# luanaruiz9/gated_gcrnns

Hardware: AMD Instinct MI355X
Metric: sequences/sec (node), N=1000 K=5 T=32 F=64 (higher is better)
Workload: dtype bf16

## Files before the change

gated_gcrnns_amd/_lib.py:

```python
import ctypes as C
import os

import torch

from . import build as _build

F32, F64, BF16 = 0, 1, 2

_c_i64 = C.c_int64
_c_p = C.c_void_p


class GcrnnError(RuntimeError):
    pass


def _load():
    path = os.environ.get('GCRNN_LIBPATH')
    if path:
        return _bind(C.CDLL(path))
    path = _build.LIBPATH
    if _build.needs_build() and os.path.exists(_build.HIPCC):
        _build.build(verbose=False)
    if not os.path.exists(path):
        raise ImportError(
            'gated_gcrnns_amd: %s is missing. Build it with `python -m gated_gcrnns_amd.build` '
            '(needs hipcc; there is no CPU fallback).' % path)
    return _bind(C.CDLL(path))


def _bind(lib):
    sig = {
        'gcrnn_version': (C.c_int, []),
        'gcrnn_status_string': (C.c_char_p, [C.c_int]),
        'gcrnn_last_hip_error': (C.c_char_p, []),
        'gcrnn_csr_count': (C.c_int, [_c_p, _c_i64, C.c_int, C.c_int, C.c_double, C.POINTER(_c_i64)]),
        'gcrnn_csr_fill': (C.c_int, [_c_p, _c_i64, C.c_int, C.c_int, C.c_double, _c_p, _c_p, _c_p]),
        'gcrnn_degree_order': (C.c_int, [_c_p, _c_i64, _c_p]),
        'gcrnn_pack_node_major': (C.c_int, [C.c_int, _c_p, _c_p, _c_i64, _c_i64, _c_i64, _c_i64, _c_p, _c_p]),
        'gcrnn_pack_node_major_sum_f32': (C.c_int, [_c_p, _c_p, _c_i64, _c_i64, _c_i64, _c_i64, _c_i64, _c_p]),
        'gcrnn_node_gate_filter_supported': (C.c_int, [_c_i64, _c_i64, _c_i64, C.c_double]),
        'gcrnn_node_gate_filter_f32': (C.c_int, [_c_p, _c_p, _c_i64, _c_i64, _c_i64, _c_i64, _c_i64, _c_i64, _c_p, _c_p, _c_p, _c_i64, C.c_double, _c_p, C.c_int, _c_p]),
        'gcrnn_unpack_node_major': (C.c_int, [C.c_int, _c_p, _c_p, _c_i64, _c_i64, _c_i64, _c_i64, _c_p, _c_p]),
        'gcrnn_spmm': (C.c_int, [C.c_int, _c_i64, _c_p, _c_p, _c_p, _c_p, _c_p, _c_i64, _c_i64, C.c_int, _c_p]),
        'gcrnn_spmm_ex': (C.c_int, [C.c_int, _c_i64, _c_p, _c_p, _c_p, _c_p, _c_p, _c_i64, _c_i64, C.c_int, _c_p, C.c_double, _c_i64,
                                    C.c_int, C.c_int, C.c_int, C.c_int, _c_p]),
        'gcrnn_taps_mfma_supported': (C.c_int, [C.c_int, _c_i64, _c_i64, _c_i64]),
        'gcrnn_taps_mfma_forward': (C.c_int, [C.c_int, _c_p, _c_p, _c_p, _c_p, _c_p, _c_p, _c_i64, _c_i64, _c_i64, _c_i64, _c_i64, _c_i64, _c_p]),
        'gcrnn_taps_bf16_supported': (C.c_int, [_c_i64, _c_i64, _c_i64]),
        'gcrnn_taps_bf16_forward': (C.c_int, [_c_p, _c_p, _c_p, _c_p, _c_p, _c_i64, _c_i64, _c_i64, _c_i64, _c_p]),
        'gcrnn_batch_time_mse_slabs': (_c_i64, [_c_i64, _c_i64]),
        'gcrnn_batch_time_mse': (C.c_int, [C.c_int, _c_p, _c_p, _c_p, _c_p, _c_i64, _c_i64, _c_p]),
        'gcrnn_adam_flat': (C.c_int, [C.c_int, _c_p, _c_p, _c_p, _c_p, _c_i64, C.c_double, C.c_double, C.c_double, C.c_double,
                                      C.c_double, _c_p, _c_p]),
        'gcrnn_adam_flat_dlr': (C.c_int, [C.c_int, _c_p, _c_p, _c_p, _c_p, _c_i64, _c_p, C.c_double, C.c_double, C.c_double,
                                          C.c_double, _c_p, _c_p]),
        'gcrnn_sgd_flat': (C.c_int, [C.c_int, _c_p, _c_p, _c_i64, _c_p, C.c_double, _c_p]),
        'gcrnn_rmsprop_flat': (C.c_int, [C.c_int, _c_p, _c_p, _c_p, _c_i64, _c_p, C.c_double, C.c_double, C.c_double, _c_p]),
        'gcrnn_taps_forward': (C.c_int, [C.c_int, _c_p, _c_p, _c_i64, _c_p, _c_p, C.c_double, _c_p,
                                         _c_i64, _c_i64, _c_i64, _c_i64, C.c_int, _c_p]),
        'gcrnn_taps_backward_data': (C.c_int, [C.c_int, _c_p, _c_p, _c_p, _c_p, _c_i64,
                                               _c_i64, _c_i64, _c_i64, _c_i64, _c_p]),
        'gcrnn_taps_backward_weight_parts': (C.c_int, [_c_i64, _c_i64, _c_i64, _c_i64, C.POINTER(_c_i64), C.POINTER(_c_i64)]),
        'gcrnn_taps_backward_weight': (C.c_int, [C.c_int, _c_p, _c_p, _c_p, _c_i64, _c_p, _c_p, C.c_double,
                                                 _c_i64, _c_i64, _c_i64, _c_i64, _c_p]),
        'gcrnn_ell_size': (C.c_int, [_c_p, _c_i64, _c_p, C.c_int, C.c_int, _c_i64, C.POINTER(_c_i64)]),
        'gcrnn_ell_fill': (C.c_int, [_c_p, _c_p, _c_p, _c_i64, _c_p, C.c_int, C.c_int, _c_i64, _c_p, _c_p, _c_p, _c_p]),
        'gcrnn_ell_assign_rows_z': (C.c_int, [_c_p, _c_p, _c_i64, _c_p, C.c_int, _c_i64, _c_i64, _c_p]),
        'gcrnn_ell_fill_z': (C.c_int, [_c_p, _c_p, _c_p, _c_i64, _c_p, C.c_int, C.c_int, _c_i64, _c_p, _c_i64, _c_p, _c_p, _c_p]),
        'gcrnn_ell_assign_rows': (C.c_int, [_c_p, _c_p, _c_i64, _c_p, C.c_int, _c_i64, _c_p]),
        'gcrnn_fused_supported': (C.c_int, [_c_i64, _c_i64, _c_i64, _c_i64]),
        'gcrnn_fused_padded_nodes': (_c_i64, []),
        'gcrnn_fused_step_waves': (_c_i64, []),
        'gcrnn_fused_wgrad_waves': (_c_i64, []),
        'gcrnn_pack_seq_major': (C.c_int, [C.c_int, _c_p, _c_p, _c_i64, _c_i64, _c_i64, _c_i64, _c_i64, _c_p, _c_p]),
        'gcrnn_pack_seq_major_padded': (C.c_int, [_c_p, _c_p] + [_c_i64] * 6 + [_c_p]),
        'gcrnn_unpack_seq_major': (C.c_int, [C.c_int, _c_p, _c_p, _c_i64, _c_i64, _c_i64, _c_i64, _c_i64, _c_p, _c_p]),
        'gcrnn_fused_pack_weights': (C.c_int, [C.c_int, _c_p, _c_p, _c_p, _c_i64, _c_i64, _c_i64, _c_i64, _c_p]),
        'gcrnn_fused_forward_bf16': (C.c_int, [_c_p, _c_p, _c_p, _c_p, _c_p, _c_p, _c_p, _c_p, _c_p, _c_p, _c_p,
                                               _c_p, _c_p,
                                               _c_i64, _c_i64, _c_i64, _c_i64, _c_i64, _c_i64, _c_i64, _c_p, C.c_int, _c_p, C.c_double, _c_p, _c_p, _c_p, _c_p]),
        'gcrnn_fused_pack_weights_wide': (C.c_int, [C.c_int, _c_p, _c_p, _c_p, _c_i64, _c_i64, _c_i64, _c_i64, _c_i64, C.c_double, _c_p]),
        'gcrnn_fused_forward_wide_supported': (C.c_int, [_c_i64] * 7 + [C.c_double, C.c_int, C.c_int]),
        'gcrnn_fused_forward_wide_bf16': (C.c_int, [_c_p] * 10 + [_c_i64] * 7 + [_c_p, C.c_int, _c_p, _c_p, _c_p, _c_p]),
        'gcrnn_fused_forward_wide_scratch_bytes': (_c_i64, [_c_i64, _c_i64, C.c_int]),
        'gcrnn_fused_forward_wide_scratch_bf16': (C.c_int, [_c_p] * 3 + [_c_i64] + [_c_p] * 7 + [_c_i64] * 7 + [_c_p, C.c_int, _c_p, _c_p, _c_p, _c_p]),
        'gcrnn_fused_forward_wide_head_supported': (C.c_int, [_c_i64] * 7 + [C.c_double, C.c_int, C.c_int]),
        'gcrnn_fused_forward_wide_head_bf16': (C.c_int, [_c_p] * 3 + [_c_i64] + [_c_p] * 7 + [_c_i64] * 7 + [_c_p] * 7),
        'gcrnn_fused_pack_weights_wide_bias': (C.c_int, [C.c_int] + [_c_p] * 5 + [_c_i64] * 5 + [C.c_double, _c_p]),
        'gcrnn_fused_forward_wide_user_bytes': (_c_i64, [_c_i64] * 3),
        'gcrnn_fused_forward_wide_user_supported': (C.c_int, [_c_i64] * 7 + [C.c_double, C.c_int]),
        'gcrnn_fused_forward_wide_user_bf16': (C.c_int, [_c_p, _c_i64, _c_p, _c_p, _c_i64] + [_c_p] * 5 + [_c_i64] * 7 + [_c_p, C.c_int, _c_p, _c_p, _c_p, _c_p]),
        'gcrnn_fused_forward_wide_head_user_supported': (C.c_int, [_c_i64] * 7 + [C.c_double, C.c_int]),
        'gcrnn_fused_forward_wide_head_user_bf16': (C.c_int, [_c_p, _c_i64, _c_p, _c_p, _c_i64] + [_c_p] * 5 + [_c_i64] * 7 + [_c_p] * 7),
        'gcrnn_fused_backward_data_wide_supported': (C.c_int, [_c_i64] * 6 + [C.c_double, C.c_int, C.c_int]),
        'gcrnn_fused_backward_data_wide_bf16': (C.c_int, [_c_p] * 8 + [_c_i64] * 6 + [_c_p] * 7),
        'gcrnn_fused_backward_data_wide_head_supported': (C.c_int, [_c_i64] * 6 + [C.c_double, C.c_int]),
        'gcrnn_fused_backward_data_wide_head_bf16': (C.c_int, [_c_p] * 9 + [_c_i64] * 6 + [_c_p] * 4),
        'gcrnn_gate_readout_finish': (C.c_int, [_c_p, _c_i64, _c_p, _c_p, _c_p, _c_p, _c_i64, _c_p]),
        'gcrnn_fused_filter_output_wide_supported': (C.c_int, [_c_i64] * 7 + [C.c_double, C.c_int, C.c_int]),
        'gcrnn_fused_filter_output_wide_bf16': (C.c_int, [_c_p] * 7 + [_c_i64] * 7 + [_c_p, _c_p]),
        'gcrnn_fused_node_forward_wide_supported': (C.c_int, [_c_i64] * 6 + [C.c_double, C.c_int]),
        'gcrnn_fused_node_forward_wide_bf16': (C.c_int, [_c_p] * 11 + [_c_i64] * 6 + [_c_p, C.c_int, _c_p]),
        'gcrnn_fused_gate_pair_wide_supported': (C.c_int, [_c_i64] * 7 + [C.c_double, C.c_int, C.c_int]),
        'gcrnn_fused_gate_pair_prepass_wide_bf16': (C.c_int, [_c_p] * 12 + [_c_i64] * 7 + [_c_p, _c_p, _c_p, _c_p]),
        'gcrnn_fused_gate_pair_prepass_taps_wide_bf16': (C.c_int, [_c_p] * 7 + [_c_i64] + [_c_p] * 5 + [_c_i64] * 7 + [_c_p, _c_p, _c_p, _c_p]),
        'gcrnn_fused_inline_pack_supported': (C.c_int, [_c_i64, _c_i64, _c_i64, _c_i64, _c_i64, C.c_double]),
        'gcrnn_fused_seq_steps_per_launch': (_c_i64, [_c_i64] * 7 + [C.c_double, C.c_int, C.c_int, C.c_int]),
        'gcrnn_fused_filter_output_bf16': (C.c_int, [_c_p] * 11 + [_c_i64] * 7 + [C.c_double, C.c_int, _c_p]),
        'gcrnn_fused_node_forward_bf16': (C.c_int, [_c_p] * 15 + [_c_i64] * 6 + [_c_p, C.c_int, C.c_double, _c_p]),
        'gcrnn_fused_node_backward_data_bf16': (C.c_int, [_c_p] * 12 + [_c_i64] * 6 + [C.c_double, _c_p, C.c_int, _c_p]),
        'gcrnn_node_cell_backward': (C.c_int, [_c_p] * 11 + [_c_i64] * 5 + [_c_p]),
        'gcrnn_node_gate_dot': (C.c_int, [_c_p, _c_p, _c_p, _c_i64, _c_i64, _c_i64, _c_i64, _c_i64, _c_p]),
        'gcrnn_node_gate_dot_backward': (C.c_int, [_c_p, _c_p, _c_p, _c_p, _c_i64, _c_i64, _c_i64, _c_i64, _c_i64, _c_p]),
        'gcrnn_fused_edge_attention_supported': (C.c_int, [_c_i64, _c_i64]),
        'gcrnn_fused_edge_attention_bf16': (C.c_int, [_c_p] * 13 + [_c_i64] * 5 + [C.c_double, _c_p]),
        'gcrnn_fused_edge_attention_backward_supported': (C.c_int, [_c_i64, _c_i64, _c_i64]),
        'gcrnn_fused_edge_attention_backward_bf16': (C.c_int, [_c_p] * 14 + [_c_i64] * 6 + [C.c_double, _c_p]),
        'gcrnn_fused_backward_step_bf16': (C.c_int, [_c_p] * 11 + [_c_i64] * 5 + [C.c_double, _c_p, _c_p, _c_i64, C.c_int, _c_p]),
        'gcrnn_fused_backward_seed_bf16': (C.c_int, [_c_p, _c_p, _c_p, _c_i64, _c_p]),
        'gcrnn_fused_x3_supported': (C.c_int, [_c_i64, _c_i64, _c_i64, _c_i64, _c_i64]),
        'gcrnn_pack_seq_major_x3': (C.c_int, [_c_p, _c_p, _c_i64, _c_i64, _c_i64, _c_i64, _c_i64, _c_p]),
        'gcrnn_fused_pack_weights_x3': (C.c_int, [_c_p, _c_p, _c_p, _c_i64, _c_i64, _c_i64, _c_i64, _c_p]),
        'gcrnn_fused_forward_x3': (C.c_int, [_c_p] * 8 + [_c_i64] * 7 + [C.c_double, _c_p, C.c_int, _c_p, _c_p]),
        'gcrnn_fused_forward_x3_scaled': (C.c_int, [_c_p] * 9 + [_c_i64] * 7 + [C.c_double, _c_p, _c_i64, _c_p, _c_p]),
        'gcrnn_fused_x3_training_supported': (C.c_int, [_c_i64] * 5),
        'gcrnn_fused_backward_data_x3': (C.c_int, [_c_p] * 8 + [_c_i64] * 6 + [C.c_double, _c_p, _c_p]),
        'gcrnn_fused_backward_weight_f32': (C.c_int, [_c_p] * 9 + [_c_i64] * 7 + [C.c_double, _c_p, _c_p]),
        'gcrnn_fused_backward_data_x3_gated': (C.c_int, [_c_p] * 8 + [_c_i64] * 6 + [C.c_double, _c_p, _c_p, _c_p, _c_p, _c_p]),
        'gcrnn_fused_filter_x3': (C.c_int, [_c_p] * 6 + [_c_i64] * 5 + [C.c_double, _c_p, _c_p]),
        'gcrnn_fused_backward_weight_f32_gated': (C.c_int, [_c_p] * 9 + [_c_i64] * 7 + [C.c_double, _c_p, _c_p, C.c_int, _c_p, _c_p]),
        'gcrnn_fused_gate_cells_x3': (C.c_int, [_c_p] * 8 + [_c_i64] * 7 + [C.c_double, _c_p, C.c_int, _c_p, _c_p]),
        'gcrnn_pack_seq_major_x3_ex': (C.c_int, [_c_p, _c_p] + [_c_i64] * 5 + [_c_p, _c_p, C.c_int, _c_i64, _c_p]),
        'gcrnn_x3_item_dots': (C.c_int, [_c_p] * 5 + [_c_i64] * 4 + [_c_p]),
        'gcrnn_x3_node_gate_step': (C.c_int, [_c_p] * 7 + [_c_i64] * 5 + [_c_p]),
        'gcrnn_pack_seq_major_steps': (C.c_int, [_c_p, _c_p, _c_i64, _c_i64, _c_i64, _c_i64, _c_i64, _c_i64, _c_i64, _c_i64, _c_p]),
        'gcrnn_fused_gate_prepass_bf16': (C.c_int, [_c_p, _c_p, _c_p, _c_p, _c_p, _c_p, _c_p, _c_p, _c_p, _c_p, _c_p, _c_p, _c_p,
                                                    _c_i64, _c_i64, _c_i64, _c_i64, _c_i64, _c_i64, _c_i64, _c_p, C.c_double, C.c_int, _c_p]),
        'gcrnn_fused_gate_prepass_pack_bf16': (C.c_int, [_c_p] * 14 + [_c_i64] * 7 + [_c_p, C.c_double, C.c_int, _c_p]),
        'gcrnn_fused_gate_prepass_lays_out': (_c_i64, [_c_i64] * 7 + [C.c_double, C.c_int]),
        'gcrnn_fused_gate_prepass_taps_bf16': (C.c_int, [_c_p] * 7 + [_c_i64] + [_c_p] * 7 + [_c_i64] * 7 + [_c_p, C.c_double, C.c_int, _c_p]),
        'gcrnn_fused_gate_prepass_taps_supported': (C.c_int, [_c_i64] * 7 + [C.c_double, C.c_int, C.c_int, _c_i64]),
        'gcrnn_fused_gate_readout_slabs': (_c_i64, [_c_i64]),
        'gcrnn_all_zero_flag_bf16': (C.c_int, [_c_p, _c_i64, _c_p, _c_p]),
        'gcrnn_fused_gate_readout_backward_bf16': (C.c_int, [_c_p, _c_p, _c_p, _c_p, _c_i64, _c_i64, _c_i64, _c_p]),
        'gcrnn_fused_gate_grad_bf16': (C.c_int, [_c_p] * 12 + [_c_i64] * 7 + [C.c_double, C.c_int, _c_p]),
        'gcrnn_fused_backward_data_bf16': (C.c_int, [_c_p, _c_p, _c_p, _c_p, _c_p, _c_p, _c_p, _c_p, _c_p, _c_p, _c_p,
                                                     _c_i64, _c_i64, _c_i64, _c_i64, _c_i64, _c_i64, _c_p, _c_p, _c_p, C.c_double, _c_p, C.c_int, _c_p]),
        'gcrnn_fused_wgrad_slots': (_c_i64, [_c_i64, _c_i64]),
        'gcrnn_fused_wgrad_bf16_slots': (_c_i64, [_c_i64, _c_i64, _c_i64, _c_i64, C.c_int]),
        'gcrnn_fused_backward_weight_bf16': (C.c_int, [_c_p, _c_p, _c_p, _c_p, _c_p, _c_p, _c_p, _c_p, _c_p, _c_p,
                                                       _c_i64, _c_i64, _c_i64, _c_i64, _c_i64, _c_i64, _c_i64, _c_p, _c_p,
                                                       C.c_int, _c_p, C.c_double, _c_p, _c_p, _c_p]),
        'gcrnn_small_supported': (C.c_int, [C.c_int, _c_i64, _c_i64, _c_i64, _c_i64, _c_i64, _c_i64]),
        'gcrnn_small_forward': (C.c_int, [C.c_int, _c_p, _c_p, _c_p, _c_p, _c_p, _c_p, _c_p, _c_p, _c_p, _c_p, _c_p,
                                          _c_i64, _c_i64, _c_i64, _c_i64, _c_i64, _c_i64, _c_i64, _c_i64, _c_p]),
        'gcrnn_small_backward_supported': (C.c_int, [C.c_int, _c_i64, _c_i64, _c_i64, _c_i64, _c_i64, _c_i64]),
        'gcrnn_small_backward': (C.c_int, [C.c_int] + [_c_p] * 21 + [_c_i64] * 8 + [_c_p]),
        'gcrnn_small_backward_dx': (C.c_int, [C.c_int] + [_c_p] * 22 + [_c_i64] * 8 + [_c_p]),
        'gcrnn_small_dense_supported': (C.c_int, [C.c_int, _c_i64, _c_i64, _c_i64, _c_i64, _c_i64, C.c_int, C.c_int]),
        'gcrnn_small_dense_forward': (C.c_int, [C.c_int] + [_c_p] * 9 + [_c_i64] * 10 + [_c_p]),
        'gcrnn_small_dense_backward': (C.c_int, [C.c_int] + [_c_p] * 16 + [_c_i64] * 10 + [_c_p]),
        'gcrnn_small_dense_backward_dx_supported': (C.c_int, [C.c_int, _c_i64, _c_i64, _c_i64, _c_i64, _c_i64, C.c_int]),
        'gcrnn_small_dense_backward_dx': (C.c_int, [C.c_int] + [_c_p] * 17 + [_c_i64] * 10 + [_c_p]),
        'gcrnn_small_dense_head_supported': (C.c_int, [C.c_int] + [_c_i64] * 6 + [C.c_int] * 3),
        'gcrnn_small_dense_forward_head': (C.c_int, [C.c_int] + [_c_p] * 12 + [_c_i64] * 11 + [C.c_int, _c_p]),
        'gcrnn_small_dense_backward_head': (C.c_int, [C.c_int] + [_c_p] * 18 + [_c_i64] * 11 + [_c_p]),
        'gcrnn_small_dense_node_head_supported': (C.c_int, [C.c_int] + [_c_i64] * 6 + [C.c_int] * 3),
        'gcrnn_small_dense_forward_node_head': (C.c_int, [C.c_int] + [_c_p] * 12 + [_c_i64] * 11 + [C.c_int, _c_p]),
        'gcrnn_small_dense_backward_node_head': (C.c_int, [C.c_int] + [_c_p] * 18 + [_c_i64] * 11 + [_c_p]),
        'gcrnn_small_dense_gnn_head_supported': (C.c_int, [C.c_int] + [_c_i64] * 6 + [C.c_int] * 3),
        'gcrnn_small_dense_forward_gnn_head': (C.c_int, [C.c_int] + [_c_p] * 12 + [_c_i64] * 11 + [C.c_int, C.c_int, _c_p]),
        'gcrnn_small_gnn_head_adjoint': (C.c_int, [C.c_int] + [_c_p] * 4 + [_c_i64] * 3 + [C.c_int, _c_p]),
        'gcrnn_small_gates_supported': (C.c_int, [C.c_int, _c_i64, _c_i64, _c_i64, _c_i64, _c_i64, C.c_int]),
        'gcrnn_small_gates_forward': (C.c_int, [C.c_int] + [_c_p] * 9 + [_c_i64] * 7 + [_c_p]),
        'gcrnn_small_gates_backward': (C.c_int, [C.c_int] + [_c_p] * 14 + [_c_i64] * 7 + [_c_p]),
        'gcrnn_small_gates_backward_dx': (C.c_int, [C.c_int] + [_c_p] * 15 + [_c_i64] * 7 + [_c_p]),
        'gcrnn_small_node_gates_supported': (C.c_int, [C.c_int, _c_i64, _c_i64, _c_i64, _c_i64, _c_i64, C.c_int]),
        'gcrnn_small_node_gates_forward': (C.c_int, [C.c_int] + [_c_p] * 9 + [_c_i64] * 7 + [_c_p]),
        'gcrnn_small_node_gates_backward': (C.c_int, [C.c_int] + [_c_p] * 14 + [_c_i64] * 7 + [_c_p]),
        'gcrnn_small_node_gates_backward_dx': (C.c_int, [C.c_int] + [_c_p] * 15 + [_c_i64] * 7 + [_c_p]),
        'gcrnn_small_edge_supported': (C.c_int, [C.c_int] + [_c_i64] * 7),
        'gcrnn_small_edge_forward': (C.c_int, [C.c_int] + [_c_p] * 21 + [_c_i64] * 9 + [C.c_int, _c_p]),
        'gcrnn_small_edge_backward_supported': (C.c_int, [C.c_int] + [_c_i64] * 7),
        'gcrnn_small_edge_backward': (C.c_int, [C.c_int] + [_c_p] * 33 + [_c_i64] * 9 + [_c_p]),
        'gcrnn_small_edge_backward_dx': (C.c_int, [C.c_int] + [_c_p] * 34 + [_c_i64] * 9 + [_c_p]),
        'gcrnn_small_edge_head_supported': (C.c_int, [C.c_int] + [_c_i64] * 7 + [C.c_int, _c_i64, C.c_int]),
        'gcrnn_small_edge_forward_head': (C.c_int, [C.c_int] + [_c_p] * 24 + [_c_i64] * 10 + [C.c_int, C.c_int, _c_p]),
        'gcrnn_small_edge_backward_head': (C.c_int, [C.c_int] + [_c_p] * 35 + [_c_i64] * 10 + [C.c_int, _c_p]),
        'gcrnn_node_linear_blocks': (_c_i64, [_c_i64, _c_i64]),
        'gcrnn_node_linear_forward': (C.c_int, [C.c_int, _c_p, _c_p, _c_p, _c_p, _c_i64, _c_i64, _c_i64, _c_i64, _c_p]),
        'gcrnn_node_linear_backward': (C.c_int, [C.c_int, _c_p, _c_p, _c_p, _c_p, _c_p, _c_p, _c_i64, _c_i64, _c_i64, _c_i64, _c_p]),
        'gcrnn_node_linear_bf16_supported': (C.c_int, [_c_i64, _c_i64, _c_i64]),
        'gcrnn_node_linear_bf16_blocks': (_c_i64, [_c_i64, _c_i64]),
        'gcrnn_node_linear_bf16_forward': (C.c_int, [C.c_int, _c_p, _c_p, _c_p, _c_p, _c_i64, _c_i64, _c_i64, _c_i64, _c_p]),
        'gcrnn_node_linear_bf16_backward': (C.c_int, [C.c_int, _c_p, _c_p, _c_p, _c_p, _c_p, _c_p, _c_i64, _c_i64, _c_i64, _c_i64, _c_p]),
        'gcrnn_graph_filter_layer_supported': (C.c_int, [C.c_int] + [_c_i64] * 6 + [C.c_int]),
        'gcrnn_graph_filter_layer_wgrad_slots': (_c_i64, [C.c_int] + [_c_i64] * 6 + [C.c_int]),
        'gcrnn_graph_filter_layer_forward': (C.c_int, [C.c_int] + [_c_p] * 7 + [C.c_double] + [_c_i64] * 7 + [C.c_int, _c_p]),
        'gcrnn_graph_filter_layer_backward': (C.c_int, [C.c_int] + [_c_p] * 7 + [_c_i64] + [_c_p] * 3 + [C.c_double] + [_c_i64] * 7
                                              + [C.c_int, _c_p]),
        'gcrnn_rnn_supported': (C.c_int, [C.c_int] + [_c_i64] * 4),
        'gcrnn_rnn_wgrad_slots': (_c_i64, [C.c_int] + [_c_i64] * 4),
        'gcrnn_rnn_forward': (C.c_int, [C.c_int] + [_c_p] * 7 + [_c_i64] * 4 + [C.c_int, _c_p]),
        'gcrnn_rnn_backward': (C.c_int, [C.c_int] + [_c_p] * 10 + [_c_i64] * 5 + [C.c_int, _c_p]),
        'gcrnn_l1_loss_blocks': (_c_i64, [_c_i64]),
        'gcrnn_l1_loss': (C.c_int, [C.c_int, _c_p, _c_p, _c_p, _c_p, _c_i64, C.c_double, _c_p]),
        'gcrnn_scale_unless_one': (C.c_int, [C.c_int, _c_p, _c_p, _c_i64, _c_p]),
        'gcrnn_cross_entropy_blocks': (_c_i64, [_c_i64, _c_i64]),
        'gcrnn_cross_entropy': (C.c_int, [C.c_int] + [_c_p] * 7 + [_c_i64, _c_i64, C.c_double, _c_p]),
        'gcrnn_attention_forward': (C.c_int, [C.c_int] + [_c_p] * 11 + [_c_i64] * 5 + [C.c_double, _c_p]),
        'gcrnn_attention_backward': (C.c_int, [C.c_int] + [_c_p] * 15 + [_c_i64] * 5 + [C.c_double, _c_p]),
        'gcrnn_ell_conflict_cycles': (C.c_int, [_c_p, _c_i64, _c_p, C.POINTER(_c_i64)]),
        'gcrnn_ell_pack_lds': (C.c_int, [_c_p, _c_p, _c_i64, _c_p, _c_p, _c_p]),
    }
    for name, (res, args) in sig.items():
        fn = getattr(lib, name)
        fn.restype = res
        fn.argtypes = args
    return lib, sorted(sig)


lib, EXPORTS = _load()


def check(status, what=''):
    if status != 0:
        detail = lib.gcrnn_last_hip_error().decode() if status == 5 else ''
        raise GcrnnError('%s failed: %s (status %d) %s' % (what or 'gcrnn call', lib.gcrnn_status_string(status).decode(),
                                                        status, detail))


def dtype_code(torch_dtype):
    import torch
    try:
        return {torch.float32: F32, torch.float64: F64, torch.bfloat16: BF16}[torch_dtype]
    except KeyError:
        raise GcrnnError('unsupported dtype %s (float32, float64, bfloat16)' % torch_dtype)
```

gated_gcrnns_amd/csrc/gcrnn_fused_seq32.h:

```cpp
#pragma once

#if defined(GCRNN_SEQ_STAMPS)
static __device__ unsigned long long gcrnn_seq32_stamps[256 * 96];
static __device__ __forceinline__ void gcrnn_stamp32_put(uint32_t lds_addr) {
  const unsigned long long tv = __builtin_amdgcn_s_memtime();
  asm volatile("ds_write_b64 %0, %1" ::"v"(lds_addr), "v"(tv) : "memory");
}
static __device__ __forceinline__ unsigned long long gcrnn_stamp32_get(uint32_t lds_addr) {
  unsigned long long tv;
  asm volatile("ds_read_b64 %0, %1\n\ts_waitcnt lgkmcnt(0)" : "=v"(tv) : "v"(lds_addr) : "memory");
  return tv;
}
#define GCRNN_STAMP32(slot)                                                                                   \
  do {                                                                                                        \
    if (wave == 0 && stamp_on && lane_now() == 0) gcrnn_stamp32_put((uint32_t)reinterpret_cast<uintptr_t>(smem) + M::FLAG_OFF + 8 * (slot)); \
  } while (0)
#define GCRNN_STAMP32_WAVE(slot0)                                                                             \
  do {                                                                                                        \
    if (stamp_on && lane_now() == 0) gcrnn_stamp32_put((uint32_t)reinterpret_cast<uintptr_t>(smem) + M::FLAG_OFF + 8 * ((slot0) + wave)); \
  } while (0)
#define GCRNN_STAMP32_FLUSH()                                                                                 \
  do {                                                                                                        \
    __syncthreads();                                                                                          \
    if (threadIdx.x < 96 && blockIdx.x < 256) gcrnn_seq32_stamps[blockIdx.x * 96 + threadIdx.x] = gcrnn_stamp32_get((uint32_t)reinterpret_cast<uintptr_t>(smem) + M::FLAG_OFF + 8 * threadIdx.x); \
  } while (0)
#ifndef GCRNN_SEQ32_STAMP_READER_NAME
#define GCRNN_SEQ32_STAMP_READER_NAME gcrnn_debug_read_seq32_stamps
#endif
extern "C" int GCRNN_SEQ32_STAMP_READER_NAME(void* host) {
  return hipMemcpyFromSymbol(host, HIP_SYMBOL(gcrnn_seq32_stamps), sizeof(unsigned long long) * 256 * 96) == hipSuccess ? 0 : 1;
}
#else
#define GCRNN_STAMP32_WAVE(slot0) do {} while (0)
#define GCRNN_STAMP32(slot) do {} while (0)
#define GCRNN_STAMP32_FLUSH() do {} while (0)
#endif

#ifndef GCRNN_SEQ32_R1_STREAM_FIRST
#define GCRNN_SEQ32_R1_STREAM_FIRST 0
#endif
#ifndef GCRNN_SEQ32_OPERAND_AT
#define GCRNN_SEQ32_OPERAND_AT 1
#endif
#ifndef GCRNN_SEQ32_NT_ROWS
#define GCRNN_SEQ32_NT_ROWS 0
#endif
#ifndef GCRNN_SEQ32_NT_DMA
#define GCRNN_SEQ32_NT_DMA 0
#endif
#ifndef GCRNN_SEQ32_NT_XLOAD
#define GCRNN_SEQ32_NT_XLOAD 0
#endif
#ifndef GCRNN_SEQ32_NT_STATE
#define GCRNN_SEQ32_NT_STATE 0
#endif
#ifndef GCRNN_SEQ32_NO_ITEM_PREFETCH
#define GCRNN_SEQ32_NO_ITEM_PREFETCH 0
#endif
#ifndef GCRNN_SEQ32_GATED_TAPS_FIRST
#define GCRNN_SEQ32_GATED_TAPS_FIRST 1
#endif
#ifndef GCRNN_SEQ32_YOUNG_PRIO
#define GCRNN_SEQ32_YOUNG_PRIO 0
#endif
#ifndef GCRNN_SEQ32_END_WAIT
#define GCRNN_SEQ32_END_WAIT 0
#endif
#ifndef GCRNN_SEQ32_SAME_ORDER
#define GCRNN_SEQ32_SAME_ORDER 0
#endif

struct Seq32Args {
  const uint16_t* x0; int64_t xstride;
  const uint16_t* hfirst;
  uint16_t* out0; int64_t ostride;
  const uint4* wpack;
  const float* bias;
  const uint16_t* a1; int64_t a1stride;
  int a1_last_only;
  int ubstride;
  const int32_t* tile_nodes; const int32_t* tile_off; const uint2* ell_col4;
  int entries, B, N;
  const uint16_t* pk_src0; int64_t pksrc_stride;
  uint16_t* pk_dst0; int64_t pkdst_stride;
  int pk_stride;
  int nsteps;
  const float* gi0; const float* gf0; int64_t gstride;
  int hmod;
  const int32_t* flags;
  const float* gw;
  const uint4* tapf; float* taps_out; int ntaps;
  float* go;
  uint16_t* out1;
  const uint16_t* dh0_; int64_t dhstride;
  const uint16_t* hs0; int64_t hsstride;
  const float* gsc0; int64_t gscstride;
  float* gpart0; int64_t gpartstride;
  int final_raw;
  uint16_t* final_out; const uint16_t* final_h;
  const float* ng0; int64_t ngstride; int64_t nghalf;
  const float* r1a; const float* r1b;
  int stagger;
  uint16_t* scr;
  const float* head_w; const float* head_b;
  float* y0;
  const uint16_t* h0u; int self_start;
  const uint16_t* dy0; int64_t dystride; int64_t dybstride;
};

__device__ __forceinline__ int lane_now() {
  int ln;
  asm volatile("v_mbcnt_lo_u32_b32 %0, -1, 0\n\tv_mbcnt_hi_u32_b32 %0, -1, %0" : "=v"(ln));
  return ln;
}

#define GCRNN_HOP_ASM_WIDE32_STREAM(D)                                                             \
  do {                                                                                             \
    const int gwbeg = tbeg[0] >> 2, gwend = tend[STILES - 1] >> 2;                                 \
    if (gwbeg < gwend) {                                                                           \
      const int ls_ = lane_now(), r = ls_ & 15, q = ls_ >> 4;                                      \
      const uint32_t colb = lds_col + r * 8 + (q >> 1) * 4;        \
      const uint32_t qh_ = (uint32_t)(q & 1) << 4;                                                 \
      asm volatile(GCRNN_HOP_ASM_WIDE32_TEXT                                                       \
                   : "+v"(D[0][0]), "+v"(D[0][1]), "+v"(D[1][0]), "+v"(D[1][1]), "+v"(D[2][0]), "+v"(D[2][1]), "+v"(D[3][0]), "+v"(D[3][1]), \
                     "+v"(D[4][0]), "+v"(D[4][1]), "+v"(D[5][0]), "+v"(D[5][1]), "+v"(D[6][0]), "+v"(D[6][1]), "+v"(D[7][0]), "+v"(D[7][1])  \
                   : "s"(GCRNN_SGPR(tend[0] >> 2)), "s"(GCRNN_SGPR(tend[1] >> 2)), "s"(GCRNN_SGPR(tend[2] >> 2)), "s"(GCRNN_SGPR(tend[3] >> 2)), \
                     "s"(GCRNN_SGPR(tend[4] >> 2)), "s"(GCRNN_SGPR(tend[5] >> 2)), "s"(GCRNN_SGPR(tend[6] >> 2)), "s"(GCRNN_SGPR(tend[7] >> 2)), \
                     "s"(GCRNN_SGPR(gwbeg)), "s"(GCRNN_SGPR(gwend - 1)), "v"(colb), "v"(qh_)               \
                   : GCRNN_HOP_ASM_WIDE32_CLOBBERS);                                               \
    }                                                                                              \
  } while (0)

template <int K, int HS, int XS>
struct Seq32Map {
  static constexpr int KS = HS + XS;
  static constexpr int PL = GCRNN_HOP_WIDE_PLANE;
  static constexpr int RS2 = 4 * NP + 16;
  static constexpr int BIAS_OFF = PL + 32 * 1024;
  static constexpr int FLAG_OFF = BIAS_OFF + 256;
  static constexpr int WOFF = 2 * PL;
  static constexpr int WB = K * KS * 2048;
  static constexpr int COL_OFF = WOFF + WB;
  static constexpr int NPCK = 128;
  static constexpr int PFS = 256;
  static_assert(16 * RS2 <= BIAS_OFF && FLAG_OFF + 768 <= WOFF, "LDS map");
  static size_t lds_bytes(int64_t entries, bool inline_pack, bool r1 = false) {
    const size_t need = (size_t)COL_OFF + (size_t)entries * 32 + GCRNN_HOP_COLUMN_PAD + NP * 4 + (r1 ? 2 * NP * 4 : 0) + (inline_pack ? (size_t)(32 * (XS > 0 ? XS : HS)) * NPCK * 2 : 0)
                        + PFS;
    return need <= 160 * 1024 ? need : 0;
  }
  static constexpr int HEAD_TAB = 512 + (HS > 1 ? NP * 4 : 0);
  static size_t lds_bytes_head(int64_t entries, bool inline_pack, bool r1 = false) {
    const size_t need = lds_bytes(entries, inline_pack, r1);
    return (need && need + HEAD_TAB <= 160 * 1024) ? need + HEAD_TAB : 0;
  }
};

template <int K, int HS, int XS, int VAR, int MODE = 0, bool GATED = false, bool R1 = false, bool SPLIT = false>
__global__ __launch_bounds__(STHREADS) void fused_seq32_kernel(const Seq32Args a) {
  static_assert(!R1 || !SPLIT, "rank-1 graphs: every mode of the persistent form (the BPTT chain takes the adjoint plan: the factors swap)");
  static_assert(!SPLIT || ((MODE == 0 || MODE == 2) && !R1 && HS > 1), "split sequences: the (un-gated or time-gated) forward and the BPTT chain, with more than one chunk");
  constexpr bool ITEMS = (MODE == 1 || MODE == 3);
  constexpr bool SONLY = (MODE == 2 || MODE == 4);
  constexpr bool PKV = (VAR & 1) != 0, USERV = (VAR & 2) != 0 && (MODE == 0 || MODE == 4);
  constexpr bool SCRV = (VAR & 4) != 0;
  constexpr bool HEADV = (VAR & 8) != 0;
  constexpr bool UPR1 = (VAR & 16) != 0;
  static_assert(!UPR1 || (VAR == 16 && MODE == 2 && !R1 && !SPLIT), "rank-1 upstream: the persistent chain on uniform-weight graphs, no inline pack");
  static_assert(!SCRV || (MODE == 0 && !SPLIT && ((VAR & 2) != 0 || HEADV)), "state scratch: the persistent forward with the user-layout output");
  static_assert(!HEADV || (SCRV && (VAR & 2) == 0), "output head: on the state scratch, no user-layout output");
  constexpr int SCR_CH = NP * 64;
  static_assert(MODE == 0 || ((MODE >= 1 && MODE <= 4) && !GATED), "modes");
  static_assert(MODE < 3 || (!R1 && !SPLIT), "modes 3, 4: uniform-weight graphs, persistent form");
  using M = Seq32Map<K, HS, XS>;
  constexpr int KS = HS + XS;
  constexpr int F = 32 * HS, G = 32 * XS;
  constexpr int NCH = (MODE == 1) ? 2 * HS : HS;
  constexpr int PL = M::PL, WOFF = M::WOFF, WB = M::WB, COL_OFF = M::COL_OFF, RS2 = M::RS2;
  constexpr int NPCK = M::NPCK, NRND = NP / NPCK, NH = NCH * (K - 1), RPH = (NRND + NH - 1) / NH;
  constexpr int PKROWS = SONLY ? F : G;
  static_assert(STILES == 8 && GCRNN_HOP_ASM && K >= 2 && (SONLY ? XS == 0 : XS > 0), "generated hop stream: 8 tiles per wave; the chain's operand is the state alone");
  extern __shared__ __attribute__((aligned(16))) char smem[];
  const int entries = a.entries, B = a.B, N = a.N;

  const int tid = threadIdx.x, lane = tid & 63;
  const int wave = __builtin_amdgcn_readfirstlane(tid >> 6);
  const int r = lane & 15, q = lane >> 4;
  constexpr int NSPL = SPLIT ? HS : 1;
  const int wg_seq = (int)blockIdx.x / NSPL, chunk0 = SPLIT ? (int)blockIdx.x % NSPL : 0, gseq = (int)gridDim.x / NSPL;
  if (wg_seq >= B) return;

  bf16x8 bfr[STILES][KS];
  constexpr bool SELFV = PKV && SCRV && MODE == 0 && !GATED && !SPLIT;
  const bool self_start = SELFV && a.self_start != 0;
  if constexpr (SELFV) {
    if (self_start) {
      constexpr int SROW = NP * 2, SPIECES = 32 * (NP / 8);
      static_assert(32 * SROW <= M::BIAS_OFF && 32 * SROW <= M::WOFF && SPIECES % STHREADS == 0 && NP / 8 == 128, "self-start staging area: below the bias table");
      const int b = wg_seq;
      const int tl = wave * 64 + lane_now();
      int nodes[STILES];
#pragma unroll
      for (int i = 0; i < STILES; ++i) nodes[i] = a.tile_nodes[(wave * STILES + i) * 16 + (tl & 15)] >> 16;
#pragma unroll
      for (int s = 0; s < KS; ++s) {
        const uint16_t* src = s < HS ? a.h0u + (int64_t)b * (F * N) + (int64_t)(32 * s) * N
                                     : a.pk_src0 + (int64_t)b * a.pk_stride + (int64_t)(32 * (s - HS)) * N;
#pragma unroll
        for (int i = 0; i < SPIECES / STHREADS; ++i) {
          const int id = i * STHREADS + tl;
          const int row = id >> 7, cs = id & 127;
          const int col = (cs - 2 * (row >> 3)) & 127;
          if (col * 8 < N)
            __builtin_amdgcn_global_load_lds((const __attribute__((address_space(1))) void*)(src + (int64_t)row * N + col * 8),
                                             (__attribute__((address_space(3))) void*)(smem + (i * STHREADS + wave * 64) * 16), 16, 0, GCRNN_SEQ32_NT_DMA);
        }
        asm volatile("s_waitcnt vmcnt(0)" ::: "memory");
        lds_barrier();
        const int qo = (tl & 63) >> 4;
#pragma unroll
        for (int i = 0; i < STILES; ++i) {
          const bool ok = nodes[i] < N;
          const int nn = ok ? nodes[i] : 0;
          const char* ra = smem + (8 * qo) * SROW + ((((nn >> 3) + 2 * qo) & 127) << 4) + (nn & 7) * 2;
          uint32_t h16[8];
#pragma unroll
          for (int j = 0; j < 8; ++j) h16[j] = *reinterpret_cast<const uint16_t*>(ra + j * SROW);
          typedef __attribute__((__vector_size__(4 * sizeof(unsigned int)))) unsigned int u32x4s_t;
          u32x4s_t v;
#pragma unroll
          for (int jj = 0; jj < 4; ++jj) v[jj] = ok ? (h16[2 * jj] | (h16[2 * jj + 1] << 16)) : 0u;
          bfr[i][s] = __builtin_bit_cast(bf16x8, v);
        }
        lds_barrier();
      }
      if (a.nsteps > 1) {
        constexpr int XN = RPH * NPCK, XROWS = G, XPPR = XN / 8, XPCS = XROWS / 8;
        static_assert(XROWS * XN * 2 <= 32 * SROW && (XROWS * XPPR) % STHREADS == 0 && (XPCS * XN) % STHREADS == 0 && XPPR >= 16, "x_1 start-up rounds");
        const __amdgpu_buffer_rsrc_t rsrc_x1 = __builtin_amdgcn_make_buffer_rsrc(a.pk_dst0 + a.pkdst_stride + (int64_t)b * (NP * G), 0, NP * G * 2, 0x00020000);
        const uint16_t* src = a.pk_src0 + (int64_t)b * a.pk_stride + a.pksrc_stride;
#pragma unroll
        for (int i = 0; i < XROWS * XPPR / STHREADS; ++i) {
          const int id = i * STHREADS + tl;
          const int row = id / XPPR, cs = id - row * XPPR;
          const int col = (cs - 2 * (row >> 3) + XPPR) % XPPR;
          if (col * 8 < N)
            __builtin_amdgcn_global_load_lds((const __attribute__((address_space(1))) void*)(src + (int64_t)row * N + col * 8),
                                             (__attribute__((address_space(3))) void*)(smem + (i * STHREADS + wave * 64) * 16), 16, 0, GCRNN_SEQ32_NT_DMA);
        }
        asm volatile("s_waitcnt vmcnt(0)" ::: "memory");
        lds_barrier();
        constexpr int XRI = XPCS * XN / STHREADS;
        typedef __attribute__((__vector_size__(4 * sizeof(unsigned int)))) unsigned int u32x4x_t;
        u32x4x_t vv[XRI];
#pragma unroll
        for (int i = 0; i < XRI; ++i) {
          const int id = i * STHREADS + tl;
          const int nl = id / XPCS, pc = id - nl * XPCS;
          const char* ra = smem + (8 * pc) * (XN * 2) + ((((nl >> 3) + 2 * pc) % XPPR) << 4) + (nl & 7) * 2;
          uint32_t h16[8];
#pragma unroll
          for (int j = 0; j < 8; ++j) h16[j] = *reinterpret_cast<const uint16_t*>(ra + j * (XN * 2));
          const bool ok = nl < N;
#pragma unroll
          for (int jj = 0; jj < 4; ++jj) vv[i][jj] = ok ? (h16[2 * jj] | (h16[2 * jj + 1] << 16)) : 0u;
        }
#pragma unroll
        for (int i = 0; i < XRI; ++i) asm volatile("" : "+v"(vv[i]));
#pragma unroll
        for (int i = 0; i < XRI; ++i) {
          const int id = i * STHREADS + tl;
          const int nl = id / XPCS, pc = id - nl * XPCS;
          __builtin_amdgcn_raw_buffer_store_b128(vv[i], rsrc_x1, nl * (G * 2) + pc * 16, 0, 0);
        }
        asm volatile("s_waitcnt vmcnt(0)" ::: "memory");
#pragma unroll
        for (int i = 0; i < XRI; ++i) asm volatile("" ::"v"(vv[i]));
        lds_barrier();
      }
    }
  }

  int tbeg[STILES], tend[STILES];
#pragma unroll
  for (int i = 0; i < STILES; ++i) {
    tbeg[i] = a.tile_off[wave * STILES + i];
    tend[i] = a.tile_off[wave * STILES + i + 1];
  }
  char* wtab = smem + COL_OFF + entries * 32 + GCRNN_HOP_COLUMN_PAD;
  for (int idx = tid; idx < NP; idx += STHREADS) reinterpret_cast<int32_t*>(wtab)[idx] = a.tile_nodes[idx];
  [[maybe_unused]] float* r1tab = reinterpret_cast<float*>(wtab + NP * 4);
  if constexpr (R1) {
    for (int idx = tid; idx < NP; idx += STHREADS) {
      const int nd = a.tile_nodes[idx] >> 16;
      r1tab[idx] = nd < NP ? a.r1a[nd] : 0.f;
      r1tab[NP + idx] = nd < NP ? a.r1b[nd] : 0.f;
    }
  }
  auto slot_words = [&](int ln, int (&w)[STILES]) {
    const uint32_t ad = (uint32_t)(COL_OFF + entries * 32 + GCRNN_HOP_COLUMN_PAD) + (uint32_t)((wave * STILES * 16 + (ln & 15)) * 4);
    asm volatile("ds_read_b32 %0, %8\n\tds_read_b32 %1, %8 offset:64\n\tds_read_b32 %2, %8 offset:128\n\tds_read_b32 %3, %8 offset:192\n\t"
                 "ds_read_b32 %4, %8 offset:256\n\tds_read_b32 %5, %8 offset:320\n\tds_read_b32 %6, %8 offset:384\n\tds_read_b32 %7, %8 offset:448\n\t"
                 "s_waitcnt lgkmcnt(0)"
                 : "=&v"(w[0]), "=&v"(w[1]), "=&v"(w[2]), "=&v"(w[3]), "=&v"(w[4]), "=&v"(w[5]), "=&v"(w[6]), "=&v"(w[7])
                 : "v"(ad));
    const int lb = (((ln >> 4) >> 1) << 4) | (((ln >> 4) & 1) << 3);
#pragma unroll
    for (int i = 0; i < STILES; ++i) w[i] ^= lb;
  };
  [[maybe_unused]] auto r1_scale = [&](f32x4 (&ac)[STILES][2], int kind) __attribute__((always_inline)) {
    if constexpr (R1) {
      const uint32_t ad = (uint32_t)(COL_OFF + entries * 32 + GCRNN_HOP_COLUMN_PAD + NP * 4 + NP * 4) + (uint32_t)((wave * STILES * 16 + (lane_now() & 15)) * 4);
      constexpr int NB = (GATED || ITEMS || K == 4) ? 1 : 4;
#pragma unroll
      for (int h4 = 0; h4 < STILES; h4 += NB) {
        float b4[NB];
        if constexpr (NB == 4)
          asm volatile("ds_read_b32 %0, %4\n\tds_read_b32 %1, %4 offset:64\n\tds_read_b32 %2, %4 offset:128\n\tds_read_b32 %3, %4 offset:192\n\t"
                       "s_waitcnt lgkmcnt(0)"
                       : "=&v"(b4[0]), "=&v"(b4[1]), "=&v"(b4[2]), "=&v"(b4[3])
                       : "v"(ad + (uint32_t)(h4 * 64)));
        else
          asm volatile("ds_read_b32 %0, %1\n\ts_waitcnt lgkmcnt(0)" : "=&v"(b4[0]) : "v"(ad + (uint32_t)(h4 * 64)));
#pragma unroll
        for (int e = 0; e < NB; ++e) {
          const float bv = b4[e];
          const float f = kind == 0 ? bv : (bv == 0.f ? 1.f : (kind == 1 ? __builtin_amdgcn_rcpf(bv) : bv));
          ac[h4 + e][0] *= f; ac[h4 + e][1] *= f;
        }
      }
    }
  };

  {
    const int cbytes = entries * 32;
    const char* csrc = reinterpret_cast<const char*>(a.ell_col4);
    for (int p = wave; p * 1024 < cbytes; p += SWAVES)
      if (p * 1024 + lane * 16 < cbytes)
        __builtin_amdgcn_global_load_lds((const __attribute__((address_space(1))) void*)(csrc + p * 1024 + lane * 16),
                                         (__attribute__((address_space(3))) void*)(smem + COL_OFF + p * 1024), 16, 0, 0);
    const char* wsrc = reinterpret_cast<const char*>(a.wpack) + (size_t)chunk0 * WB;
    for (int p = wave; p < WB / 1024; p += SWAVES)
      __builtin_amdgcn_global_load_lds((const __attribute__((address_space(1))) void*)(wsrc + p * 1024 + lane * 16),
                                       (__attribute__((address_space(3))) void*)(smem + WOFF + p * 1024), 16, 0, 0);
    asm volatile("s_waitcnt vmcnt(0)" ::: "memory");
  }
  if (tid < GCRNN_HOP_COLUMN_PAD / 4) reinterpret_cast<uint32_t*>(smem + COL_OFF + entries * 32)[tid] = 0u;
  float* lbias = reinterpret_cast<float*>(smem + M::BIAS_OFF);
  if constexpr (UPR1) {
    if (tid < F) lbias[tid] = a.head_w[tid];
  } else
  if (tid < NCH * 32) lbias[tid] = a.bias ? a.bias[tid] : 0.f;
  if constexpr (HEADV) {
    float* ht = reinterpret_cast<float*>(smem + COL_OFF + entries * 32 + GCRNN_HOP_COLUMN_PAD + NP * 4 + (R1 ? 2 * NP * 4 : 0));
    if (tid < F) ht[tid] = a.head_w[tid];
    if (tid == F) ht[64] = a.head_b ? a.head_b[0] : 0.f;
  }
  __syncthreads();

  if (a.stagger > 0) {
    const unsigned long long t0 = __builtin_amdgcn_s_memtime();
    const unsigned long long d = (unsigned long long)((blockIdx.x >> 3) & 7) * (unsigned long long)a.stagger;
    while (__builtin_amdgcn_s_memtime() - t0 < d) __builtin_amdgcn_s_sleep(16);
  }
  const uint32_t lds0 = (uint32_t)reinterpret_cast<uintptr_t>(smem);
  if (lds0 != 0) __builtin_trap();
  const uint32_t lds_col = lds0 + COL_OFF;
  [[maybe_unused]] float* htab = reinterpret_cast<float*>(wtab + NP * 4 + (R1 ? 2 * NP * 4 : 0));
  char* xtile = wtab + NP * 4 + (R1 ? 2 * NP * 4 : 0) + (HEADV ? M::HEAD_TAB : 0);

  const int skip_hi = __builtin_amdgcn_readfirstlane((MODE == 3 || (MODE == 1 && a.flags && a.flags[0] != 0)) ? 1 : 0);
  const bool skip_h = skip_hi != 0;
  auto load_first_operand = [&](int b) {
    const __amdgpu_buffer_rsrc_t rsrc_h = __builtin_amdgcn_make_buffer_rsrc(const_cast<uint16_t*>(a.hfirst), 0, skip_h ? 0 : (ITEMS ? a.hmod : B) * (NP * F * 2), 0x00020000);
    const __amdgpu_buffer_rsrc_t rsrc_x = __builtin_amdgcn_make_buffer_rsrc(const_cast<uint16_t*>(a.x0), 0, XS > 0 ? B * (NP * G * 2) : 0, 0x00020000);
    const int bh = ITEMS ? __builtin_amdgcn_readfirstlane(b % a.hmod) : b;
    const int ln0 = lane_now(), qo = ln0 >> 4;
    int sw[STILES];
    slot_words(ln0, sw);
#pragma unroll
    for (int s = 0; s < KS; ++s) {
#pragma unroll
      for (int i = 0; i < STILES; ++i) {
        const int w = sw[i];
        if (s < HS)
          bfr[i][s] = __builtin_bit_cast(bf16x8, __builtin_amdgcn_raw_buffer_load_b128(rsrc_h, (w >> 16) * (F * 2) + 16 * qo + 64 * s, bh * (NP * F * 2), 0));
        else
          bfr[i][s] = __builtin_bit_cast(bf16x8, __builtin_amdgcn_raw_buffer_load_b128(rsrc_x, (w >> 16) * (G * 2) + 16 * qo + 64 * (s - HS), b * (NP * G * 2), 0));
      }
    }
  };
  bool have_operand = self_start;
  for (int b = wg_seq; b < B; b += gseq) {
  if (!have_operand) load_first_operand(b);
  have_operand = false;
#pragma unroll 1
  for (int step = 0; step < a.nsteps; ++step) {
    const bool fin = (MODE == 2) && a.final_raw && step == a.nsteps - 1;
    uint16_t* hout = fin ? a.final_out : (a.out0 ? a.out0 + (int64_t)step * a.ostride : nullptr);
    [[maybe_unused]] const uint16_t* ep_dh = (SONLY && !fin && a.dh0_) ? a.dh0_ + (int64_t)step * a.dhstride : nullptr;
    [[maybe_unused]] const float* ep_ng = (MODE == 4) ? a.ng0 + (int64_t)step * a.ngstride : nullptr;
    [[maybe_unused]] const uint16_t* ep_h = (MODE == 2) ? (fin ? a.final_h : (a.hs0 ? a.hs0 + (int64_t)step * a.hsstride : nullptr)) : nullptr;
    [[maybe_unused]] const uint16_t* ep_dy = (UPR1 && !fin && a.dy0) ? a.dy0 + (int64_t)step * a.dystride + (int64_t)b * a.dybstride : nullptr;
    [[maybe_unused]] const bool ep_up = UPR1 ? ep_dy != nullptr : ep_dh != nullptr;
    [[maybe_unused]] float* gpart = (MODE == 2 && a.gpart0) ? a.gpart0 + (int64_t)step * a.gpartstride : nullptr;
    [[maybe_unused]] float gsc = 1.f;
    if constexpr (MODE == 2) {
      if (a.gsc0) gsc = __builtin_bit_cast(float, __builtin_amdgcn_readfirstlane(__builtin_bit_cast(int, a.gsc0[(int64_t)step * a.gscstride + b])));
    }
    float gin = 1.f, gfo = 1.f, gratio = 1.f;
    if constexpr (MODE == 4) {
      if (a.gi0) {
        gin = __builtin_bit_cast(float, __builtin_amdgcn_readfirstlane(__builtin_bit_cast(int, a.gi0[(int64_t)step * a.gstride + b])));
        gfo = __builtin_bit_cast(float, __builtin_amdgcn_readfirstlane(__builtin_bit_cast(int, a.gf0[(int64_t)step * a.gstride + b])));
      }
    }
    if constexpr (GATED) {
      gin = __builtin_bit_cast(float, __builtin_amdgcn_readfirstlane(__builtin_bit_cast(int, a.gi0[(int64_t)step * a.gstride + b])));
      gfo = __builtin_bit_cast(float, __builtin_amdgcn_readfirstlane(__builtin_bit_cast(int, a.gf0[(int64_t)step * a.gstride + b])));
      gratio = __builtin_bit_cast(float, __builtin_amdgcn_readfirstlane(__builtin_bit_cast(int, gfo / fmaxf(gin, 1e-30f))));
    }
    const uint16_t* aux1 = (USERV && a.a1) ? (a.a1_last_only ? (step == a.nsteps - 1 ? a.a1 : nullptr) : a.a1 + (int64_t)step * a.a1stride) : nullptr;
    const bool pk_any = PKV && a.pk_src0 != nullptr;
    const int ubstride = a.ubstride;
    const int nb = b + (int)gridDim.x;
    const int nbq = ITEMS ? __builtin_amdgcn_readfirstlane(nb / a.hmod) : 0, nbr = ITEMS ? __builtin_amdgcn_readfirstlane(nb - nbq * a.hmod) : 0;
    const int64_t pk_soff = ITEMS ? (int64_t)nbr * a.pk_stride + (int64_t)nbq * a.pksrc_stride : (int64_t)b * a.pk_stride;
    const int pk_db = ITEMS ? nb : b;
    const __amdgpu_buffer_rsrc_t rsrc_o = __builtin_amdgcn_make_buffer_rsrc(hout, 0, hout ? B * (NP * F * 2) : 0, 0x00020000);
    [[maybe_unused]] const bool stamp_on = (step == (a.nsteps > 2 ? a.nsteps - 3 : 0)) && b == wg_seq;
    GCRNN_STAMP32(0);
    const bool more = step + 1 < a.nsteps;
    const __amdgpu_buffer_rsrc_t rsrc_xn = __builtin_amdgcn_make_buffer_rsrc(const_cast<uint16_t*>(XS > 0 ? a.x0 + (int64_t)(step + 1) * a.xstride : nullptr), 0, (more && XS > 0) ? B * (NP * G * 2) : 0, 0x00020000);

    f32x4 acc[STILES][2];
    auto taps = [&](int tap, [[maybe_unused]] bool on_sums = false) {
#ifdef GCRNN_SEQ32_EXPERIMENT_NO_HOP_TAPS
      if (tap != K - 1) return;
#endif
      const int ln = lane_now();
      const uint32_t wofs = (uint32_t)WOFF + (uint32_t)ln * 16u;
      if constexpr (GATED) {
        const bool xpart = gin > 1e-30f;
        const bool hpart = !on_sums || gfo > 1e-30f;
        if (on_sums) {
          const float pre = hpart ? 1.f / gfo : (xpart ? 1.f / gin : 1.f);
#pragma unroll
          for (int i = 0; i < STILES; ++i) { acc[i][0] *= pre; acc[i][1] *= pre; }
        }
#pragma unroll
        for (int h = 0; h < 2; ++h) {
          if (hpart) {
#pragma unroll
            for (int s = 0; s < HS; ++s) {
              const bf16x8 afr = __builtin_bit_cast(bf16x8, *reinterpret_cast<const uint4*>(smem + wofs + (uint32_t)(((tap * 2 + h) * KS + s) * 1024)));
#pragma unroll
              for (int i = 0; i < STILES; ++i) acc[i][h] = __builtin_amdgcn_mfma_f32_16x16x32_bf16(afr, bfr[i][s], acc[i][h], 0, 0, 0);
            }
          }
          if (hpart) {
#pragma unroll
            for (int i = 0; i < STILES; ++i) acc[i][h] *= (xpart ? gratio : gfo);
          }
          if (xpart) {
#pragma unroll
            for (int s = HS; s < KS; ++s) {
              const bf16x8 afr = __builtin_bit_cast(bf16x8, *reinterpret_cast<const uint4*>(smem + wofs + (uint32_t)(((tap * 2 + h) * KS + s) * 1024)));
#pragma unroll
              for (int i = 0; i < STILES; ++i) acc[i][h] = __builtin_amdgcn_mfma_f32_16x16x32_bf16(afr, bfr[i][s], acc[i][h], 0, 0, 0);
            }
            if constexpr (GATED) {
#pragma unroll
              for (int i = 0; i < STILES; ++i) acc[i][h] *= gin;
            }
          }
        }
      } else if constexpr (ITEMS) {
#pragma unroll
        for (int h = 0; h < 2; ++h)
#pragma unroll
          for (int s = 0; s < KS; ++s) {
            if (s < HS && skip_h) continue;
            const bf16x8 afr = __builtin_bit_cast(bf16x8, *reinterpret_cast<const uint4*>(smem + wofs + (uint32_t)(((tap * 2 + h) * KS + s) * 1024)));
#pragma unroll
            for (int i = 0; i < STILES; ++i) acc[i][h] = __builtin_amdgcn_mfma_f32_16x16x32_bf16(afr, bfr[i][s], acc[i][h], 0, 0, 0);
          }
      } else {
      uint4 af[2];
      af[0] = *reinterpret_cast<const uint4*>(smem + wofs + (uint32_t)((tap * 2 * KS) * 1024));
#pragma unroll
      for (int hs = 0; hs < 2 * KS; ++hs) {
        const int h = hs / KS, s = hs - h * KS;
        if (hs + 1 < 2 * KS) af[(hs + 1) & 1] = *reinterpret_cast<const uint4*>(smem + wofs + (uint32_t)((tap * 2 * KS + hs + 1) * 1024));
        const bf16x8 afr = __builtin_bit_cast(bf16x8, af[hs & 1]);
#pragma unroll
        for (int i = 0; i < STILES; ++i) acc[i][h] = __builtin_amdgcn_mfma_f32_16x16x32_bf16(afr, bfr[i][s], acc[i][h], 0, 0, 0);
      }
      }
    };
    auto put = [&](auto tpc) __attribute__((always_inline)) {
      constexpr bool tprime = decltype(tpc)::value;
      int sw[STILES];
      slot_words(lane_now(), sw);
#pragma unroll
      for (int i = 0; i < STILES; ++i) {
        const int wv = sw[i];
        if constexpr (R1) {
          const int slot = (wave * STILES + i) * 16 + (lane_now() & 15);
          float av = r1tab[slot];
          if constexpr (tprime) { const float bv = r1tab[NP + slot]; av *= (bv == 0.f ? 1.f : bv); }
          state_put<true>(reinterpret_cast<float*>(smem), wv, acc[i][0] * av);
          state_put<true>(reinterpret_cast<float*>(smem + PL), wv, acc[i][1] * av);
        } else {
          state_put<true>(reinterpret_cast<float*>(smem), wv, acc[i][0]);
          state_put<true>(reinterpret_cast<float*>(smem + PL), wv, acc[i][1]);
        }
      }
    };
    auto seed = [&]() {
#pragma unroll
      for (int i = 0; i < STILES; ++i) { acc[i][0] = f32x4{0.f, 0.f, 0.f, 0.f}; acc[i][1] = f32x4{0.f, 0.f, 0.f, 0.f}; }
      taps(K - 1);
      put(std::false_type{});
    };
    auto seed_taps_beside_rows = [&]() {
#pragma unroll
      for (int i = 0; i < STILES; ++i) { acc[i][0] = f32x4{0.f, 0.f, 0.f, 0.f}; acc[i][1] = f32x4{0.f, 0.f, 0.f, 0.f}; }
      taps(K - 1);
    };
    seed();

#pragma unroll 1
    for (int chunk = chunk0; chunk < (SPLIT ? chunk0 + 1 : NCH); ++chunk) {
      const bool last = SPLIT || chunk == NCH - 1;
      lds_barrier();
      GCRNN_STAMP32(1 + chunk * 24);

      auto pack_target = [&](int v, int& tgt, int& rnd) -> bool {
        if constexpr (ITEMS) {
          rnd = v; tgt = 0;
          return pk_any && v < NRND && nb < B;
        }
        if constexpr (SPLIT) {
          rnd = v; tgt = 0;
          return pk_any && v < NRND;
        }
        if constexpr (MODE == 2) {
          rnd = v; tgt = step + 1;
          return pk_any && v < NRND && tgt < a.nsteps - (a.final_raw ? 1 : 0);
        }
        v += RPH;
        const int wrap = v >= NRND ? 1 : 0;
        rnd = v - wrap * NRND;
        tgt = step + 1 + wrap;
        return pk_any && tgt >= (self_start ? 1 : 2) && tgt < a.nsteps;
      };
      auto pack_issue = [&](int v) {
        int tgt, rnd;
        if (!pack_target(v, tgt, rnd)) return;
        const uint16_t* pk_src = a.pk_src0 + ((ITEMS || SPLIT) ? 0 : (int64_t)tgt * a.pksrc_stride);
        constexpr int PPR = NPCK / 8, PIECES = PKROWS * PPR;
        static_assert(PIECES % STHREADS == 0, "whole pieces per thread");
        const uint16_t* xsrc = pk_src + pk_soff + rnd * NPCK;
        const int tl = wave * 64 + lane_now();
#pragma unroll
        for (int i = 0; i < PIECES / STHREADS; ++i) {
          const int id = i * STHREADS + tl;
          const int row = id / PPR, cs = id - row * PPR;
          const int col = (cs - (row >> 3)) & (PPR - 1);
          if (rnd * NPCK + col * 8 < N)
            __builtin_amdgcn_global_load_lds((const __attribute__((address_space(1))) void*)(xsrc + (int64_t)row * N + col * 8),
                                             (__attribute__((address_space(3))) void*)(xtile + (i * STHREADS + wave * 64) * 16), 16, 0, GCRNN_SEQ32_NT_DMA);
        }
      };
      auto pack_drain = [&](int v) {
        int tgt, rnd;
        if (!pack_target(v, tgt, rnd)) return;
        uint16_t* pk_dst = a.pk_dst0 + ((ITEMS || SPLIT) ? 0 : (int64_t)tgt * a.pkdst_stride);
        constexpr int PCS = PKROWS / 8, RI = PCS * NPCK / STHREADS;
        static_assert(PCS * NPCK % STHREADS == 0, "whole row pieces per thread");
        typedef __attribute__((__vector_size__(4 * sizeof(unsigned int)))) unsigned int u32x4_t;
        const __amdgpu_buffer_rsrc_t rsrc_pk = __builtin_amdgcn_make_buffer_rsrc(pk_dst, 0, B * (NP * PKROWS * 2), 0x00020000);
        const int tl = wave * 64 + lane_now();
        u32x4_t vv[RI];
        static_assert(RI == 1 || RI == 2, "one or two row pieces per thread");
        uint32_t h16[RI][8];
        uint32_t sa[RI];
#pragma unroll
        for (int i = 0; i < RI; ++i) {
          const int id = i * STHREADS + tl;
          const int nl = id / PCS, pc = id - nl * PCS;
          sa[i] = (uint32_t)(xtile - smem) + (uint32_t)((pc * 8) * (NPCK * 2) + ((nl + 8 * pc) & (NPCK - 1)) * 2);
        }
        static_assert(NPCK * 2 == 256, "row pitch of the pack tile in the asm offsets");
        if constexpr (RI == 2) {
          asm volatile("ds_read_u16 %0, %16\n\tds_read_u16 %1, %16 offset:256\n\tds_read_u16 %2, %16 offset:512\n\tds_read_u16 %3, %16 offset:768\n\t"
                       "ds_read_u16 %4, %16 offset:1024\n\tds_read_u16 %5, %16 offset:1280\n\tds_read_u16 %6, %16 offset:1536\n\tds_read_u16 %7, %16 offset:1792\n\t"
                       "ds_read_u16 %8, %17\n\tds_read_u16 %9, %17 offset:256\n\tds_read_u16 %10, %17 offset:512\n\tds_read_u16 %11, %17 offset:768\n\t"
                       "ds_read_u16 %12, %17 offset:1024\n\tds_read_u16 %13, %17 offset:1280\n\tds_read_u16 %14, %17 offset:1536\n\tds_read_u16 %15, %17 offset:1792\n\t"
                       "s_waitcnt lgkmcnt(0)"
                       : "=&v"(h16[0][0]), "=&v"(h16[0][1]), "=&v"(h16[0][2]), "=&v"(h16[0][3]), "=&v"(h16[0][4]), "=&v"(h16[0][5]), "=&v"(h16[0][6]), "=&v"(h16[0][7]),
                         "=&v"(h16[RI - 1][0]), "=&v"(h16[RI - 1][1]), "=&v"(h16[RI - 1][2]), "=&v"(h16[RI - 1][3]), "=&v"(h16[RI - 1][4]), "=&v"(h16[RI - 1][5]), "=&v"(h16[RI - 1][6]), "=&v"(h16[RI - 1][7])
                       : "v"(sa[0]), "v"(sa[RI - 1]));
        } else {
          asm volatile("ds_read_u16 %0, %8\n\tds_read_u16 %1, %8 offset:256\n\tds_read_u16 %2, %8 offset:512\n\tds_read_u16 %3, %8 offset:768\n\t"
                       "ds_read_u16 %4, %8 offset:1024\n\tds_read_u16 %5, %8 offset:1280\n\tds_read_u16 %6, %8 offset:1536\n\tds_read_u16 %7, %8 offset:1792\n\t"
                       "s_waitcnt lgkmcnt(0)"
                       : "=&v"(h16[0][0]), "=&v"(h16[0][1]), "=&v"(h16[0][2]), "=&v"(h16[0][3]), "=&v"(h16[0][4]), "=&v"(h16[0][5]), "=&v"(h16[0][6]), "=&v"(h16[0][7])
                       : "v"(sa[0]));
        }
#pragma unroll
        for (int i = 0; i < RI; ++i) {
          const int id = i * STHREADS + tl;
          const int nl = id / PCS;
          const bool ok = rnd * NPCK + nl < N;
          uint32_t w4[4];
#pragma unroll
          for (int jj = 0; jj < 4; ++jj) w4[jj] = h16[i][2 * jj] | (h16[i][2 * jj + 1] << 16);
          vv[i] = u32x4_t{ok ? w4[0] : 0u, ok ? w4[1] : 0u, ok ? w4[2] : 0u, ok ? w4[3] : 0u};
        }
#pragma unroll
        for (int i = 0; i < RI; ++i) asm volatile("" : "+v"(vv[i]));
#pragma unroll
        for (int i = 0; i < RI; ++i) {
          const int id = i * STHREADS + tl;
          const int nl = id / PCS, pc = id - nl * PCS;
          __builtin_amdgcn_raw_buffer_store_b128(vv[i], rsrc_pk, (rnd * NPCK + nl) * (PKROWS * 2) + pc * 16 + pk_db * (NP * PKROWS * 2), 0, 0);
        }
      };

      auto r0_of = [&](int j) { return (chunk * (K - 1) + (j - 1)) * RPH; };
      auto weights_issue = [&](int wc, int tap) {
        const char* wsrc = reinterpret_cast<const char*>(a.wpack) + (size_t)wc * WB + (size_t)tap * (2 * KS * 1024);
        const int lane = lane_now();
#pragma unroll
        for (int i = 0; i < (2 * KS + SWAVES - 1) / SWAVES; ++i) {
          const int piece = i * SWAVES + wave;
          if (piece < 2 * KS)
            __builtin_amdgcn_global_load_lds((const __attribute__((address_space(1))) void*)(wsrc + piece * 1024 + lane * 16),
                                             (__attribute__((address_space(3))) void*)(smem + WOFF + tap * (2 * KS * 1024) + piece * 1024), 16, 0, 0);
        }
      };
      typedef __attribute__((__vector_size__(4 * sizeof(unsigned int)))) unsigned int u32x4e_t;
      [[maybe_unused]] u32x4e_t eph[MODE == 2 ? STILES : 1], epg[(SONLY && !UPR1) ? STILES : 1];
      [[maybe_unused]] uint32_t epy[UPR1 ? STILES : 1];
      [[maybe_unused]] float epn[MODE == 4 ? STILES : 1][2];
#ifndef GCRNN_SEQ32_EP_FIRST
#define GCRNN_SEQ32_EP_FIRST 1
#endif
#ifndef GCRNN_SEQ32_EP_EARLY
#define GCRNN_SEQ32_EP_EARLY 0
#endif
      constexpr int EPH = (SONLY && K >= 4 && !GCRNN_SEQ32_EP_EARLY) ? K - 2 : 0;
      auto ep_request = [&](auto i0c, auto i1c) __attribute__((always_inline)) {
        if constexpr (MODE == 4) {
          constexpr int I0 = decltype(i0c)::value, I1 = decltype(i1c)::value;
          const int lq = lane_now();
          int swp[STILES];
          slot_words(lq, swp);
          const __amdgpu_buffer_rsrc_t rsrc_eg = __builtin_amdgcn_make_buffer_rsrc(const_cast<uint16_t*>(ep_dh), 0, ep_dh ? B * (NP * F * 2) : 0, 0x00020000);
          const __amdgpu_buffer_rsrc_t rsrc_n = __builtin_amdgcn_make_buffer_rsrc(const_cast<float*>(ep_ng), 0, (int)(a.nghalf * 8), 0x00020000);
#pragma unroll
          for (int i = I0; i < I1; ++i) {
            const int node = swp[i] >> 16;
            epg[i] = __builtin_amdgcn_raw_buffer_load_b128(rsrc_eg, node * (F * 2) + (chunk * 32 + (lq >> 4) * 8) * 2, b * (NP * F * 2), 0);
            const int go = node < N ? (b * N + node) * 4 : 0x7ffffff0;
            epn[i][0] = __builtin_bit_cast(float, __builtin_amdgcn_raw_buffer_load_b32(rsrc_n, go, 0, 0));
            epn[i][1] = __builtin_bit_cast(float, __builtin_amdgcn_raw_buffer_load_b32(rsrc_n, go, (int)(a.nghalf * 4), 0));
          }
        }
        if constexpr (MODE == 2) {
          constexpr int I0 = decltype(i0c)::value, I1 = decltype(i1c)::value;
          const int lq = lane_now();
          int swp[STILES];
          slot_words(lq, swp);
          const __amdgpu_buffer_rsrc_t rsrc_eh = __builtin_amdgcn_make_buffer_rsrc(const_cast<uint16_t*>(ep_h), 0, ep_h ? B * (NP * F * 2) : 0, 0x00020000);
          const __amdgpu_buffer_rsrc_t rsrc_eg = UPR1 ? __builtin_amdgcn_make_buffer_rsrc(const_cast<uint16_t*>(ep_dy), 0, ep_dy ? N * 2 : 0, 0x00020000)
                                                      : __builtin_amdgcn_make_buffer_rsrc(const_cast<uint16_t*>(ep_dh), 0, ep_dh ? B * (NP * F * 2) : 0, 0x00020000);
#pragma unroll
          for (int i = I0; i < I1; ++i) {
            const int eoff = (swp[i] >> 16) * (F * 2) + (chunk * 32 + (lq >> 4) * 8) * 2;
            eph[i] = __builtin_amdgcn_raw_buffer_load_b128(rsrc_eh, eoff, b * (NP * F * 2), 0);
            if constexpr (UPR1) epy[i] = __builtin_amdgcn_raw_buffer_load_b16(rsrc_eg, (swp[i] >> 16) * 2, 0, 0);
            else epg[i] = __builtin_amdgcn_raw_buffer_load_b128(rsrc_eg, eoff, b * (NP * F * 2), 0);
          }
        }
      };
      if constexpr (SONLY && EPH == 0) ep_request(std::integral_constant<int, 0>{}, std::integral_constant<int, STILES>{});
      auto hop = [&](auto jc) __attribute__((always_inline)) {
        constexpr int j = decltype(jc)::value;
        auto dma_issue = [&]() {
          if (NCH > 1 && !SPLIT) {
            weights_issue((chunk + 1) % NCH, K - j);
            if (j == 1 && K > 2) weights_issue(chunk, 0);
          }
          if (r0_of(j) < NRND) pack_issue(r0_of(j));
        };
        const int r0 = r0_of(j);
#pragma unroll
        for (int i = 0; i < STILES; ++i) { acc[i][0] = f32x4{0.f, 0.f, 0.f, 0.f}; acc[i][1] = f32x4{0.f, 0.f, 0.f, 0.f}; }
        const bool stream_first = (!GATED || !GCRNN_SEQ32_GATED_TAPS_FIRST) && (wave < SWAVES / 2 || GCRNN_SEQ32_SAME_ORDER || (R1 && GCRNN_SEQ32_R1_STREAM_FIRST));
        if (stream_first) {
          dma_issue();
          GCRNN_HOP_ASM_WIDE32_STREAM(acc);
          r1_scale(acc, 0);
          GCRNN_STAMP32(1 + chunk * 24 + 4 * (j - 1) + 1);
          if (j == 2 && chunk == 0) GCRNN_STAMP32_WAVE(56);
          taps(K - 1 - j, true);
        } else {
          taps(K - 1 - j);
          r1_scale(acc, 1);
          if (j == 2 && chunk == 0) GCRNN_STAMP32_WAVE(56);
          dma_issue();
#if GCRNN_SEQ32_YOUNG_PRIO
          __builtin_amdgcn_s_setprio(GCRNN_SEQ32_YOUNG_PRIO);
#endif
          GCRNN_HOP_ASM_WIDE32_STREAM(acc);
#if GCRNN_SEQ32_YOUNG_PRIO
          __builtin_amdgcn_s_setprio(0);
#endif
        }
        GCRNN_STAMP32(1 + chunk * 24 + 4 * (j - 1) + 2);
        if (j == 2 && chunk == 0) GCRNN_STAMP32_WAVE(64);
        if (pk_any || (NCH > 1 && !SPLIT)) asm volatile("s_waitcnt vmcnt(0)" ::: "memory");
        lds_barrier();
        GCRNN_STAMP32(1 + chunk * 24 + 4 * (j - 1) + 3);
#if GCRNN_SEQ32_EP_FIRST
        if constexpr (SONLY && EPH > 0 && j <= EPH)
          ep_request(std::integral_constant<int, (j - 1) * STILES / (EPH > 0 ? EPH : 1)>{}, std::integral_constant<int, j * STILES / (EPH > 0 ? EPH : 1)>{});
#endif
        if (j < K - 1) {
          if (R1 && !stream_first) put(std::true_type{});
          else put(std::false_type{});
        }
        if constexpr (R1 && j == K - 1) {
          if (!stream_first) r1_scale(acc, 2);
        }
        if (K == 2 && NCH > 1 && !SPLIT) weights_issue((chunk + 1) % NCH, 0);
        if (r0 < NRND) pack_drain(r0);
#pragma unroll
        for (int e = 1; e < RPH; ++e) {
          if (pk_any && r0 + e < NRND) {
            lds_barrier();
            pack_issue(r0 + e);
            asm volatile("s_waitcnt vmcnt(0)" ::: "memory");
            lds_barrier();
            pack_drain(r0 + e);
          }
        }
#if !GCRNN_SEQ32_EP_FIRST
        if constexpr (SONLY && EPH > 0 && j <= EPH)
          ep_request(std::integral_constant<int, (j - 1) * STILES / (EPH > 0 ? EPH : 1)>{}, std::integral_constant<int, j * STILES / (EPH > 0 ? EPH : 1)>{});
#endif
        if (j < K - 1) lds_barrier();
        GCRNN_STAMP32(1 + chunk * 24 + 4 * (j - 1) + 4);
      };
      seq_static_for(hop, std::make_integer_sequence<int, K - 1>{});

      typedef __attribute__((__vector_size__(4 * sizeof(unsigned int)))) unsigned int u32x4_t;
      const int lane = lane_now(), q = lane >> 4;
      auto scratch_rsrc = [&]() {
        return __builtin_amdgcn_make_buffer_rsrc(SCRV ? a.scr + (int64_t)blockIdx.x * ((HS - 1) * (SCR_CH / 2)) : nullptr, 0, SCRV ? (HS - 1) * SCR_CH : 0, 0x00020000);
      };
      auto request_next_operand = [&]() {
        if (ITEMS || !(last && more)) return;
        const int qo = lane_now() >> 4;
        int sw[STILES];
        slot_words(lane, sw);
        const __amdgpu_buffer_rsrc_t rsrc_hn = __builtin_amdgcn_make_buffer_rsrc(SCRV ? nullptr : hout, 0, SCRV ? 0 : B * (NP * F * 2), 0x00020000);
        [[maybe_unused]] const __amdgpu_buffer_rsrc_t rsrc_sn = scratch_rsrc();
#pragma unroll
        for (int s = 0; s < KS; ++s) {
          if (s == HS - 1) continue;
#pragma unroll
          for (int i = 0; i < STILES; ++i) {
            const int w = sw[i];
#ifdef GCRNN_SEQ32_EXPERIMENT_SKIP
            if ((GCRNN_SEQ32_EXPERIMENT_SKIP == 1) == (s < HS)) continue;
#endif
            if (SCRV && s < HS)
              bfr[i][s] = __builtin_bit_cast(bf16x8, __builtin_amdgcn_raw_buffer_load_b128(rsrc_sn, (lane_now() & 15) * 64 + 16 * qo, s * SCR_CH + (wave * STILES + i) * 1024, 16));
            else if (s < HS)
              bfr[i][s] = __builtin_bit_cast(bf16x8, __builtin_amdgcn_raw_buffer_load_b128(rsrc_hn, (w >> 16) * (F * 2) + 16 * qo + 64 * s, b * (NP * F * 2), GCRNN_SEQ32_NT_XLOAD));
            else
              bfr[i][s] = __builtin_bit_cast(bf16x8, __builtin_amdgcn_raw_buffer_load_b128(rsrc_xn, (w >> 16) * (G * 2) + 16 * qo + 64 * (s - HS), b * (NP * G * 2), GCRNN_SEQ32_NT_XLOAD));
          }
        }
      };
      if (GCRNN_SEQ32_OPERAND_AT == 0) request_next_operand();
      if (ITEMS) GCRNN_STAMP32(1 + chunk * 24 + 19);
      float bs[2][4];
#pragma unroll
      for (int h = 0; h < 2; ++h)
#pragma unroll
        for (int e = 0; e < 4; ++e) bs[h][e] = (MODE >= 3 ? 1.f : (gin + gfo)) * lbias[chunk * 32 + q * 8 + h * 4 + e];
      u32x4_t pkd[STILES];
      int swe[STILES];
      slot_words(lane, swe);
      if constexpr (MODE == 1) {
        const int gate = chunk / HS, cg = chunk - gate * HS;
        if (a.tapf) {
          typedef __attribute__((__vector_size__(4 * sizeof(unsigned int)))) unsigned int u32x4t;
          const uint4* tfp = a.tapf + ((size_t)(gate * HS + cg) * 3) * 64 + lane;
          bf16x8 ta[3];
#pragma unroll
          for (int pl = 0; pl < 3; ++pl) ta[pl] = __builtin_bit_cast(bf16x8, tfp[pl * 64]);
          const __amdgpu_buffer_rsrc_t rsrc_c = __builtin_amdgcn_make_buffer_rsrc(gate ? a.out1 : a.out0, 0, (gate ? a.out1 : a.out0) ? B * (NP * F * 2) : 0, 0x00020000);
          float* so = a.taps_out + (((int64_t)b * 2 + gate) * HS + cg) * (int64_t)a.ntaps * N;
#pragma unroll
          for (int i = 0; i < STILES; ++i) {
            const int node = swe[i] >> 16;
            u32x4t p{0u, 0u, 0u, 0u};
            if (node < N) {
              const f32x4 a0 = acc[i][0], a1 = acc[i][1];
              p[0] = pack2bf(fast_tanh(a0[0] + bs[0][0]), fast_tanh(a0[1] + bs[0][1]));
              p[1] = pack2bf(fast_tanh(a0[2] + bs[0][2]), fast_tanh(a0[3] + bs[0][3]));
              p[2] = pack2bf(fast_tanh(a1[0] + bs[1][0]), fast_tanh(a1[1] + bs[1][1]));
              p[3] = pack2bf(fast_tanh(a1[2] + bs[1][2]), fast_tanh(a1[3] + bs[1][3]));
            }
            if (gate ? a.out1 : a.out0) __builtin_amdgcn_raw_buffer_store_b128(p, rsrc_c, node * (F * 2) + (cg * 32 + q * 8) * 2, b * (NP * F * 2), 0);
            f32x4 d = {0.f, 0.f, 0.f, 0.f};
#pragma unroll
            for (int pl = 2; pl >= 0; --pl) d = __builtin_amdgcn_mfma_f32_16x16x32_bf16(ta[pl], __builtin_bit_cast(bf16x8, p), d, 0, 0, 0);
            if (node < N) {
#pragma unroll
              for (int e = 0; e < 4; ++e)
                if (q * 4 + e < a.ntaps) so[(int64_t)(q * 4 + e) * N + node] = d[e];
            }
          }
        } else {
        const float* gwp = a.gw + (int64_t)gate * N * F + cg * 32 + q * 8;
        uint16_t* cso = gate ? a.out1 : a.out0;
        const __amdgpu_buffer_rsrc_t rsrc_c = __builtin_amdgcn_make_buffer_rsrc(cso, 0, cso ? B * (NP * F * 2) : 0, 0x00020000);
        float part = 0.f;
#ifndef GCRNN_SEQ32_GATE_W_PIPELINE
#define GCRNN_SEQ32_GATE_W_PIPELINE 1
#endif
        float4 w8s[2][2][2];
        auto w8_load = [&](int set, int i0l) __attribute__((always_inline)) {
#pragma unroll
          for (int t2 = 0; t2 < 2; ++t2) {
            const int nd = (swe[i0l + t2] >> 16) < N ? (swe[i0l + t2] >> 16) : N - 1;
            w8s[set][t2][0] = *reinterpret_cast<const float4*>(gwp + (int64_t)nd * F);
            w8s[set][t2][1] = *reinterpret_cast<const float4*>(gwp + (int64_t)nd * F + 4);
          }
        };
        if (GCRNN_SEQ32_GATE_W_PIPELINE) w8_load(0, 0);
#pragma unroll
        for (int i0 = 0; i0 < STILES; i0 += 2) {
          const int wset = GCRNN_SEQ32_GATE_W_PIPELINE ? (i0 >> 1) & 1 : 0;
          if (GCRNN_SEQ32_GATE_W_PIPELINE) { if (i0 + 2 < STILES) w8_load(wset ^ 1, i0 + 2); }
          else w8_load(0, i0);
          const auto& w8 = w8s[wset];
#pragma unroll
          for (int t2 = 0; t2 < 2; ++t2) {
            const int i = i0 + t2;
            const int node = swe[i] >> 16;
            u32x4_t p{0u, 0u, 0u, 0u};
            if (node < N) {
              const f32x4 a0 = acc[i][0], a1 = acc[i][1];
              const float o0 = fast_tanh(a0[0] + bs[0][0]), o1 = fast_tanh(a0[1] + bs[0][1]), o2 = fast_tanh(a0[2] + bs[0][2]), o3 = fast_tanh(a0[3] + bs[0][3]);
              const float o4 = fast_tanh(a1[0] + bs[1][0]), o5 = fast_tanh(a1[1] + bs[1][1]), o6 = fast_tanh(a1[2] + bs[1][2]), o7 = fast_tanh(a1[3] + bs[1][3]);
              part = __builtin_fmaf(o3, w8[t2][0].w, __builtin_fmaf(o2, w8[t2][0].z, __builtin_fmaf(o1, w8[t2][0].y, __builtin_fmaf(o0, w8[t2][0].x, part))));
              part = __builtin_fmaf(o7, w8[t2][1].w, __builtin_fmaf(o6, w8[t2][1].z, __builtin_fmaf(o5, w8[t2][1].y, __builtin_fmaf(o4, w8[t2][1].x, part))));
              p[0] = pack2bf(o0, o1); p[1] = pack2bf(o2, o3); p[2] = pack2bf(o4, o5); p[3] = pack2bf(o6, o7);
            }
            if (cso) __builtin_amdgcn_raw_buffer_store_b128(p, rsrc_c, node * (F * 2) + (cg * 32 + q * 8) * 2, b * (NP * F * 2), 0);
          }
        }
        GCRNN_STAMP32(1 + chunk * 24 + 18);
#pragma unroll
        for (int off = 32; off > 0; off >>= 1) part += __shfl_down(part, off, 64);
        if (lane == 0) a.go[(int64_t)b * (NCH * SWAVES) + chunk * SWAVES + wave] = part;
        }
      } else if constexpr (MODE == 3) {
        const __amdgpu_buffer_rsrc_t rsrc_c = __builtin_amdgcn_make_buffer_rsrc(a.out0, 0, B * (NP * F * 2), 0x00020000);
#pragma unroll
        for (int i = 0; i < STILES; ++i) {
          const int node = swe[i] >> 16;
          u32x4_t p{0u, 0u, 0u, 0u};
          if (node < N) {
            const f32x4 a0 = acc[i][0], a1 = acc[i][1];
            p[0] = pack2bf(a0[0] + bs[0][0], a0[1] + bs[0][1]); p[1] = pack2bf(a0[2] + bs[0][2], a0[3] + bs[0][3]);
            p[2] = pack2bf(a1[0] + bs[1][0], a1[1] + bs[1][1]); p[3] = pack2bf(a1[2] + bs[1][2], a1[3] + bs[1][3]);
          }
          __builtin_amdgcn_raw_buffer_store_b128(p, rsrc_c, node * (F * 2) + (chunk * 32 + q * 8) * 2, b * (NP * F * 2), 0);
        }
      } else if constexpr (MODE == 4) {
#pragma unroll
        for (int i = 0; i < STILES; ++i) {
          const int node = swe[i] >> 16;
          u32x4_t p{0u, 0u, 0u, 0u};
          if (node < N) {
            const float ni = gin * epn[i][0], nf = gfo * epn[i][1];
            float yv[8], rw[8];
#pragma unroll
            for (int e = 0; e < 4; ++e) {
              yv[2 * e] = bf2f((uint16_t)(epg[i][e] & 0xffffu)); yv[2 * e + 1] = bf2f((uint16_t)(epg[i][e] >> 16));
              rw[e] = acc[i][0][e] + bs[0][e]; rw[4 + e] = acc[i][1][e] + bs[1][e];
            }
            float o[8];
#pragma unroll
            for (int e = 0; e < 8; ++e) o[e] = fast_tanh(ni * yv[e] + nf * rw[e]);
            p[0] = pack2bf(o[0], o[1]); p[1] = pack2bf(o[2], o[3]); p[2] = pack2bf(o[4], o[5]); p[3] = pack2bf(o[6], o[7]);
          }
          pkd[i] = p;
          __builtin_amdgcn_raw_buffer_store_b128(p, rsrc_o, node * (F * 2) + (chunk * 32 + q * 8) * 2, b * (NP * F * 2), 0);
        }
      } else if constexpr (MODE == 2) {
        float part = 0.f;
        [[maybe_unused]] float hw8[8];
        if constexpr (UPR1) {
#pragma unroll
          for (int e = 0; e < 8; ++e) hw8[e] = lbias[chunk * 32 + q * 8 + e];
        }
#pragma unroll
        for (int i = 0; i < STILES; ++i) {
          const int node = swe[i] >> 16;
          float hv[8], gv[8], rw[8];
#pragma unroll
          for (int e = 0; e < 4; ++e) {
            hv[2 * e] = bf2f((uint16_t)(eph[i][e] & 0xffffu)); hv[2 * e + 1] = bf2f((uint16_t)(eph[i][e] >> 16));
            if constexpr (!UPR1) { gv[2 * e] = bf2f((uint16_t)(epg[i][e] & 0xffffu)); gv[2 * e + 1] = bf2f((uint16_t)(epg[i][e] >> 16)); }
            rw[e] = acc[i][0][e]; rw[4 + e] = acc[i][1][e];
          }
          if constexpr (UPR1) {
            const float dyv = bf2f((uint16_t)epy[i]);
#pragma unroll
            for (int e = 0; e < 8; ++e) gv[e] = bf2f(f2bf(hw8[e] * dyv));
          }
          if (gpart) {
#pragma unroll
            for (int e = 0; e < 8; ++e) part = __builtin_fmaf(rw[e], hv[e], part);
          }
          float o[8];
#pragma unroll
          for (int e = 0; e < 8; ++e) {
            o[e] = rw[e] * gsc;
            if (ep_up) o[e] = (o[e] + gv[e]) * (1.f - hv[e] * hv[e]);
          }
          u32x4_t p{0u, 0u, 0u, 0u};
          if (node < N) { p[0] = pack2bf(o[0], o[1]); p[1] = pack2bf(o[2], o[3]); p[2] = pack2bf(o[4], o[5]); p[3] = pack2bf(o[6], o[7]); }
          pkd[i] = p;
          __builtin_amdgcn_raw_buffer_store_b128(p, rsrc_o, node * (F * 2) + (chunk * 32 + q * 8) * 2, b * (NP * F * 2), 0);
        }
        if (gpart) {
#pragma unroll
          for (int off = 32; off > 0; off >>= 1) part += __shfl_down(part, off, 64);
          if (lane == 0) gpart[(int64_t)b * (NCH * SWAVES) + chunk * SWAVES + wave] = part;
        }
      } else {
#pragma unroll
      for (int i = 0; i < STILES; ++i) {
        const int node = swe[i] >> 16;
        u32x4_t p{0u, 0u, 0u, 0u};
        if (node < N) {
          const f32x4 a0 = acc[i][0], a1 = acc[i][1];
          p[0] = pack2bf(fast_tanh(a0[0] + bs[0][0]), fast_tanh(a0[1] + bs[0][1]));
          p[1] = pack2bf(fast_tanh(a0[2] + bs[0][2]), fast_tanh(a0[3] + bs[0][3]));
          p[2] = pack2bf(fast_tanh(a1[0] + bs[1][0]), fast_tanh(a1[1] + bs[1][1]));
          p[3] = pack2bf(fast_tanh(a1[2] + bs[1][2]), fast_tanh(a1[3] + bs[1][3]));
        }
        pkd[i] = p;
        if constexpr (HEADV) {
          const float4* hwp = reinterpret_cast<const float4*>(htab + chunk * 32 + q * 8);
          const float4 hw0 = hwp[0], hw1 = hwp[1];
          float ys = __builtin_bit_cast(float, p[0] << 16) * hw0.x;
          ys = __builtin_fmaf(hw0.y, __builtin_bit_cast(float, p[0] & 0xffff0000u), ys);
          ys = __builtin_fmaf(hw0.z, __builtin_bit_cast(float, p[1] << 16), ys);
          ys = __builtin_fmaf(hw0.w, __builtin_bit_cast(float, p[1] & 0xffff0000u), ys);
          ys = __builtin_fmaf(hw1.x, __builtin_bit_cast(float, p[2] << 16), ys);
          ys = __builtin_fmaf(hw1.y, __builtin_bit_cast(float, p[2] & 0xffff0000u), ys);
          ys = __builtin_fmaf(hw1.z, __builtin_bit_cast(float, p[3] << 16), ys);
          ys = __builtin_fmaf(hw1.w, __builtin_bit_cast(float, p[3] & 0xffff0000u), ys);
          ys += __shfl_xor(ys, 16, 64);
          ys += __shfl_xor(ys, 32, 64);
          if (q == 0) {
            float* yp = htab + 128 + (wave * STILES + i) * 16 + lane;
            if (HS > 1 && chunk > 0) ys = *yp + ys;
            if (HS > 1 && !last) *yp = ys;
            if (last && node < N) {
              const __amdgpu_buffer_rsrc_t rsrc_y = __builtin_amdgcn_make_buffer_rsrc(a.y0 + ((int64_t)b * a.nsteps + step) * N, 0, N * 4, 0x00020000);
              __builtin_amdgcn_raw_buffer_store_b32(__builtin_bit_cast(unsigned int, ys + htab[64]), rsrc_y, node * 4, 0, 0);
            }
          }
        }
        if constexpr (SCRV) {
          if (!last) __builtin_amdgcn_raw_buffer_store_b128(p, scratch_rsrc(), (lane & 15) * 64 + 16 * q, chunk * SCR_CH + (wave * STILES + i) * 1024, 0);
        } else
        if (GCRNN_SEQ32_NT_STATE && last) __builtin_amdgcn_raw_buffer_store_b128(p, rsrc_o, node * (F * 2) + (chunk * 32 + q * 8) * 2, b * (NP * F * 2), GCRNN_SEQ32_NT_STATE);
        else __builtin_amdgcn_raw_buffer_store_b128(p, rsrc_o, node * (F * 2) + (chunk * 32 + q * 8) * 2, b * (NP * F * 2), 0);
        static_assert(!SCRV || GCRNN_SEQ32_OPERAND_AT != 3, "state scratch: the per-tile request form reads the state image");
        if (GCRNN_SEQ32_OPERAND_AT == 3 && last && more) {
          const __amdgpu_buffer_rsrc_t rsrc_hn = __builtin_amdgcn_make_buffer_rsrc(hout, 0, B * (NP * F * 2), 0x00020000);
#pragma unroll
          for (int s = 0; s < KS; ++s) {
            if (s == HS - 1) continue;
            if (s < HS)
              bfr[i][s] = __builtin_bit_cast(bf16x8, __builtin_amdgcn_raw_buffer_load_b128(rsrc_hn, node * (F * 2) + 16 * q + 64 * s, b * (NP * F * 2), 0));
            else
              bfr[i][s] = __builtin_bit_cast(bf16x8, __builtin_amdgcn_raw_buffer_load_b128(rsrc_xn, node * (G * 2) + 16 * q + 64 * (s - HS), b * (NP * G * 2), 0));
          }
        }
      }
      }
      GCRNN_STAMP32(1 + chunk * 24 + 17);
      if (!ITEMS && last) {
#pragma unroll
        for (int i = 0; i < STILES; ++i) bfr[i][HS - 1] = __builtin_bit_cast(bf16x8, pkd[i]);
      }
      if (GCRNN_SEQ32_OPERAND_AT == 1) request_next_operand();
      if constexpr (ITEMS) {
        if (last && b + (int)gridDim.x < B && !GCRNN_SEQ32_NO_ITEM_PREFETCH) {
          load_first_operand(b + (int)gridDim.x);
          have_operand = true;
        }
      }
      if (aux1) {
        char* tst = smem;
        int swt[STILES];
        slot_words(lane, swt);
#pragma unroll
        for (int i = 0; i < STILES; ++i) {
          const int node = swt[i] >> 16;
          char* ra = tst + (4 * q) * RS2 + node * 4;
#pragma unroll
          for (int k = 0; k < 4; ++k) *reinterpret_cast<uint32_t*>(ra + k * RS2) = pkd[i][k];
        }
        lds_barrier();
        GCRNN_STAMP32(1 + chunk * 24 + 18);
      }
      constexpr bool OVL = USERV && MODE == 0 && !GATED && !SPLIT;
      const bool ovl = OVL && chunk + 1 < NCH;
      if (ovl && wave < SWAVES / 2) {
        seed_taps_beside_rows();
        GCRNN_STAMP32(1 + chunk * 24 + 21);
      }
      if (aux1) {
        const char* tst = smem;
        const int segs = N >> 3;
        uint16_t* ub = const_cast<uint16_t*>(aux1) + (int64_t)b * ubstride + (int64_t)(chunk * 32) * N;
        const __amdgpu_buffer_rsrc_t rsrc_u = __builtin_amdgcn_make_buffer_rsrc(ub, 0, 32 * N * 2, 0x00020000);
        static_assert(SWAVES * 2 == 16 && 128 * 32 <= RS2, "row stores: two feature-pair rows per wave, two sweeps of 64 segments inside a tile row");
        const int ln = lane_now();
        const char* rb = tst + (2 * wave) * RS2 + ln * 32;
        u32x4_t rw[4][2], rv[4][2];
#pragma unroll
        for (int p = 0; p < 4; ++p) {
          rw[p][0] = *reinterpret_cast<const u32x4_t*>(rb + (p & 1) * RS2 + (p >> 1) * 2048);
          rw[p][1] = *reinterpret_cast<const u32x4_t*>(rb + (p & 1) * RS2 + (p >> 1) * 2048 + 16);
        }
#pragma unroll
        for (int p = 0; p < 4; ++p) {
          const u32x4_t w0 = rw[p][0], w1 = rw[p][1];
          rv[p][0] = u32x4_t{__builtin_amdgcn_perm(w0[1], w0[0], 0x05040100u), __builtin_amdgcn_perm(w0[3], w0[2], 0x05040100u),
                             __builtin_amdgcn_perm(w1[1], w1[0], 0x05040100u), __builtin_amdgcn_perm(w1[3], w1[2], 0x05040100u)};
          rv[p][1] = u32x4_t{__builtin_amdgcn_perm(w0[1], w0[0], 0x07060302u), __builtin_amdgcn_perm(w0[3], w0[2], 0x07060302u),
                             __builtin_amdgcn_perm(w1[1], w1[0], 0x07060302u), __builtin_amdgcn_perm(w1[3], w1[2], 0x07060302u)};
        }
#pragma unroll
        for (int p = 0; p < 4; ++p) { asm volatile("" : "+v"(rv[p][0])); asm volatile("" : "+v"(rv[p][1])); }
#pragma unroll
        for (int p = 0; p < 4; ++p) {
          const int fp = 2 * wave + (p & 1), sg = ln + 64 * (p >> 1);
          if (sg < segs) {
            __builtin_amdgcn_raw_buffer_store_b128(rv[p][0], rsrc_u, ((2 * fp) * N + sg * 8) * 2, 0, GCRNN_SEQ32_NT_ROWS);
            __builtin_amdgcn_raw_buffer_store_b128(rv[p][1], rsrc_u, ((2 * fp + 1) * N + sg * 8) * 2, 0, GCRNN_SEQ32_NT_ROWS);
          }
        }
      }
      if (ovl && wave >= SWAVES / 2) seed_taps_beside_rows();
      if (GCRNN_SEQ32_OPERAND_AT == 2) request_next_operand();
      GCRNN_STAMP32(1 + chunk * 24 + 19);
      if (K == 2 && NCH > 1 && !SPLIT) asm volatile("s_waitcnt vmcnt(0)" ::: "memory");
      else if (GCRNN_SEQ32_END_WAIT) asm volatile("s_waitcnt vmcnt(0)" ::: "memory");
      lds_barrier();
      GCRNN_STAMP32(1 + chunk * 24 + 20);
      if (!SPLIT && chunk + 1 < NCH) {
        if (ovl) put(std::false_type{});
        else seed();
      }
    }
  }
  }
  GCRNN_STAMP32_FLUSH();
}
```

gated_gcrnns_amd/csrc/gcrnn_fused_seq32s.hip:

```cpp
#include "gcrnn_fused_step.h"
#define GCRNN_SEQ32_STAMP_READER_NAME gcrnn_debug_read_seq32s_stamps
#include "gcrnn_fused_seq32.h"

template <int K, int HS, int XS, int VAR, bool GATED, bool R1>
static int seq32s_launch_v(const Seq32Args& sa, size_t lds, hipStream_t st) {
  static_assert((VAR & 6) == 6, "state scratch: with the user-layout output");
  auto sk = fused_seq32_kernel<K, HS, XS, VAR, 0, GATED, R1>;
  if (hipFuncSetAttribute(reinterpret_cast<const void*>(sk), hipFuncAttributeMaxDynamicSharedMemorySize, (int)lds) != hipSuccess)
    return GCRNN_ERR_LAUNCH;
  GCRNN_PRE_LAUNCH();
  sk<<<(unsigned)((sa.B < gcrnn_persistent_grid() || sa.self_start) ? sa.B : gcrnn_persistent_grid()), STHREADS, lds, st>>>(sa);
  GCRNN_CHECK_LAUNCH();
  return GCRNN_OK;
}

template <int K, int HS, int XS>
static int seq32s_launch(const Seq32Args& sa, bool inline_pack, size_t lds, hipStream_t st) {
  if (!sa.a1 || (HS > 1 && !sa.scr)) return GCRNN_ERR_NULL_POINTER;
  if (sa.gi0) {
    if (inline_pack) return GCRNN_ERR_BAD_SHAPE;
    return sa.r1a ? seq32s_launch_v<K, HS, XS, 6, true, true>(sa, lds, st) : seq32s_launch_v<K, HS, XS, 6, true, false>(sa, lds, st);
  }
  if (sa.r1a) return inline_pack ? seq32s_launch_v<K, HS, XS, 7, false, true>(sa, lds, st) : seq32s_launch_v<K, HS, XS, 6, false, true>(sa, lds, st);
  return inline_pack ? seq32s_launch_v<K, HS, XS, 7, false, false>(sa, lds, st) : seq32s_launch_v<K, HS, XS, 6, false, false>(sa, lds, st);
}

int gcrnn_seq32s_forward(const Seq32Args& sa, int K, int HS, int XS, bool inline_pack, size_t lds, hipStream_t st) {
#define GCRNN_SEQ32S_CASE(KK, HH, XX) if (K == KK && HS == HH && XS == XX) return seq32s_launch<KK, HH, XX>(sa, inline_pack, lds, st);
  GCRNN_SEQ32S_CASE(5, 2, 2) GCRNN_SEQ32S_CASE(4, 2, 2) GCRNN_SEQ32S_CASE(3, 2, 2) GCRNN_SEQ32S_CASE(2, 2, 2)
  GCRNN_SEQ32S_CASE(5, 2, 1) GCRNN_SEQ32S_CASE(4, 2, 1) GCRNN_SEQ32S_CASE(3, 2, 1) GCRNN_SEQ32S_CASE(2, 2, 1)
  GCRNN_SEQ32S_CASE(5, 1, 1) GCRNN_SEQ32S_CASE(4, 1, 1) GCRNN_SEQ32S_CASE(3, 1, 1) GCRNN_SEQ32S_CASE(2, 1, 1)
#undef GCRNN_SEQ32S_CASE
  return GCRNN_ERR_UNSUPPORTED;
}
```

include/gcrnn.h:

```cpp
#ifndef GCRNN_H
#define GCRNN_H

#include <stdint.h>

#ifdef __cplusplus
extern "C" {
#endif

enum { GCRNN_F32 = 0, GCRNN_F64 = 1, GCRNN_BF16 = 2 };

enum {
  GCRNN_OK = 0,
  GCRNN_ERR_BAD_DTYPE = 1,
  GCRNN_ERR_BAD_SHAPE = 2,
  GCRNN_ERR_NULL_POINTER = 3,
  GCRNN_ERR_UNSUPPORTED = 4,
  GCRNN_ERR_LAUNCH = 5,
  GCRNN_ERR_WORKSPACE = 6
};

int gcrnn_version(void);
const char* gcrnn_status_string(int status);
const char* gcrnn_last_hip_error(void);

int gcrnn_csr_count(const double* S, int64_t N, int transpose, int add_identity, double tol, int64_t* nnz);
int gcrnn_csr_fill(const double* S, int64_t N, int transpose, int add_identity, double tol,
                   int32_t* rowptr, int32_t* col, double* val);
int gcrnn_degree_order(const int32_t* rowptr, int64_t N, int32_t* order);

int gcrnn_pack_node_major(int dtype, const void* src, void* dst, int64_t B, int64_t T, int64_t C, int64_t N,
                          const int32_t* perm, void* stream);
int gcrnn_pack_node_major_sum_f32(const void* src, void* dst, int64_t B, int64_t S, int64_t T, int64_t C, int64_t N, void* stream);
int gcrnn_node_gate_filter_supported(int64_t K, int64_t N, int64_t nnz, double uniform_w);
int gcrnn_node_gate_filter_f32(const void* parts, void* out, int64_t items, int64_t S, int64_t K, int64_t N, int64_t groups, int64_t B,
                               const int32_t* rowptr, const int32_t* col, const void* val, int64_t nnz, double uniform_w, const void* bias,
                               int sigmoid, void* stream);
int gcrnn_unpack_node_major(int dtype, const void* src, void* dst, int64_t B, int64_t T, int64_t C, int64_t N,
                            const int32_t* perm, void* stream);

int gcrnn_spmm(int dtype, int64_t N, const int32_t* rowptr, const int32_t* col, const void* val,
               const void* X, void* Y, int64_t L, int64_t nbatch, int accumulate, void* stream);
int gcrnn_spmm_ex(int dtype, int64_t N, const int32_t* rowptr, const int32_t* col, const void* val, const void* X, void* Y,
                  int64_t L, int64_t nbatch, int accumulate, const void* bias, double bias_scale, int64_t F, int act,
                  int piece_lanes, int unroll, int rows_per_wave, void* stream);
int gcrnn_taps_mfma_supported(int dtype, int64_t F, int64_t Ch, int64_t Cx);
int gcrnn_taps_mfma_forward(int dtype, const void* zh, const void* zx, const void* wB, const void* wA, void* out0, void* outrest,
                            int64_t R, int64_t F, int64_t Ch, int64_t Cx, int64_t Kst, int64_t Kin, void* stream);
int gcrnn_taps_bf16_supported(int64_t F, int64_t G, int64_t K);
int gcrnn_taps_bf16_forward(const void* zh, const void* zx, const void* wpack, void* out0, void* outrest, int64_t R,
                            int64_t F, int64_t G, int64_t K, void* stream);

int gcrnn_taps_forward(int dtype, const void* z0, const void* zrest, int64_t zstride, const void* w,
                       const void* bias, double bias_scale, void* y, int64_t rows, int64_t KK, int64_t G,
                       int64_t F, int accumulate, void* stream);
int gcrnn_taps_backward_data(int dtype, const void* dy, const void* w, void* dz0, void* dzrest, int64_t zstride,
                             int64_t rows, int64_t KK, int64_t G, int64_t F, void* stream);
int gcrnn_taps_backward_weight_parts(int64_t rows, int64_t KK, int64_t G, int64_t F, int64_t* splits, int64_t* bias_blocks);
int gcrnn_taps_backward_weight(int dtype, const void* dy, const void* z0, const void* zrest, int64_t zstride,
                               void* dw_part, void* dbias_part, double bias_scale, int64_t rows, int64_t KK, int64_t G,
                               int64_t F, void* stream);

int gcrnn_ell_size(const int32_t* rowptr, int64_t N, const int32_t* order, int tile, int pad, int64_t ntiles,
                   int64_t* nentries);
int gcrnn_ell_fill(const int32_t* rowptr, const int32_t* col, const double* val, int64_t N, const int32_t* order,
                   int tile, int pad, int64_t ntiles, const int32_t* node_addr, int32_t* tile_off, int32_t* ell_col,
                   float* ell_val);
int gcrnn_fused_filter_output_bf16(const void* zs, const void* xs, const void* wpack, const float* bias, void* out,
                                   const int32_t* tile_nodes, const int32_t* tile_off, const int32_t* ell_col, const float* ell_val,
                                   const void* ell_val4, const void* ell_col4, int64_t entries, int64_t B, int64_t T, int64_t N,
                                   int64_t F, int64_t G, int64_t K, double uniform_w, int img16 ,
                                   void* stream);
int gcrnn_fused_node_forward_bf16(const void* h0s, void* hs, const void* yx, const float* ngates, const float* gi, const float* gf,
                                  const void* wpackB, const float* bias, void* yh_out, const int32_t* tile_nodes,
                                  const int32_t* tile_off, const int32_t* ell_col, const float* ell_val, const void* ell_val4,
                                  const void* ell_col4, int64_t entries, int64_t B, int64_t T, int64_t N, int64_t F, int64_t K,
                                  void* Huser, int huser_last_only, double uniform_w, void* stream);
int gcrnn_fused_node_backward_data_bf16(const void* dHs, const void* hs, void* dpre, void* dyh, const float* ngf, const void* wpackT,
                                        const int32_t* tile_nodes, const int32_t* tile_off, const int32_t* ell_col,
                                        const float* ell_val, const void* ell_val4, const void* ell_col4, int64_t entries, int64_t B,
                                        int64_t T, int64_t N, int64_t F, int64_t K, double uniform_w,
                                        const void* dHuser_inline , int img16 , void* stream);
int gcrnn_node_cell_backward(const void* dpre, const void* yx, const void* yh, const float* ngates, const float* gi, const float* gf,
                             void* dyx, float* dni, float* dnf, float* dgi, float* dgf, int64_t B, int64_t T, int64_t N,
                             int64_t NPad, int64_t F, void* stream);
int gcrnn_node_gate_dot(const void* d, const float* w, float* s, int64_t items, int64_t N, int64_t NPad, int64_t F, int64_t K,
                        void* stream);
int gcrnn_node_gate_dot_backward(void* d, const float* ds, const float* w, float* dw_part, int64_t items, int64_t N, int64_t NPad,
                                 int64_t F, int64_t K, void* stream);

int gcrnn_fused_edge_attention_supported(int64_t N, int64_t F);
int gcrnn_fused_edge_attention_bf16(const void* z, const float* a12, const void* gx, const float* gi, const float* gf,
                                    const int32_t* rowptr, const void* r_edge, const int32_t* t_rowptr, const void* t_edge,
                                    const int32_t* t_order, void* out_seq, void* r_out, void* Huser, int64_t huser_item_stride, int64_t items, int64_t N,
                                    int64_t NPad, int64_t F, double negative_slope, void* stream);

int gcrnn_fused_edge_attention_backward_supported(int64_t N, int64_t F, int64_t max_out_degree);
int gcrnn_fused_edge_attention_backward_bf16(const void* dpre, const void* r, const float* g, const void* z, const float* a12,
                                             const int32_t* rowptr, const void* r_edge, const int32_t* r_order,
                                             const int32_t* t_rowptr, const int32_t* t_pos, float* scratch, void* dz, float* da_part,
                                             float* dgate, int64_t items, int64_t N, int64_t NPad, int64_t F, int64_t nnz,
                                             int64_t max_out_degree ,
                                             double negative_slope, void* stream);
int gcrnn_fused_backward_step_bf16(const void* operand, const void* dH_prev, const void* h_prev, void* dpre_prev, const void* wpackT,
                                   const int32_t* tile_nodes, const int32_t* tile_off, const int32_t* ell_col, const float* ell_val,
                                   const void* ell_val4, const void* ell_col4, int64_t entries, int64_t B, int64_t N, int64_t F,
                                   int64_t K, double uniform_w,
                                   const void* dHuser_next , void* dHs_next ,
                                   int64_t T ,
                                   int img16 , void* stream);
int gcrnn_fused_backward_seed_bf16(const void* dH, const void* h, void* dpre, int64_t elements, void* stream);

int gcrnn_fused_x3_supported(int64_t N, int64_t F, int64_t G, int64_t K, int64_t entries);
int gcrnn_pack_seq_major_x3(const void* src, void* dst, int64_t B, int64_t T, int64_t C, int64_t N, int64_t NPad, void* stream);
int gcrnn_fused_pack_weights_x3(const void* wA, const void* wB, void* wpack3, int64_t F, int64_t G, int64_t Kin, int64_t Kst,
                                void* stream);
int gcrnn_fused_forward_x3(const void* xs3, const void* h03, void* hs3, const void* wpack3, const float* bias,
                           const int32_t* tile_nodes, const int32_t* tile_off, const void* ell_col4, int64_t entries, int64_t B,
                           int64_t T, int64_t N, int64_t F, int64_t G, int64_t K, double uniform_w, void* Huser, int last_only,
                           const float* rank1, void* stream);
int gcrnn_fused_forward_x3_scaled(const void* xs3, const void* h03, void* hs3, const void* wpack3, const float* bias,
                                  const float* bias_scale, const int32_t* tile_nodes, const int32_t* tile_off, const void* ell_col4,
                                  int64_t entries, int64_t B, int64_t T, int64_t N, int64_t F, int64_t G, int64_t K, double uniform_w,
                                  void* Huser, int64_t huser_seq_stride, const float* rank1, void* stream);
int gcrnn_fused_x3_training_supported(int64_t N, int64_t F, int64_t G, int64_t K, int64_t entries_adj);
int gcrnn_fused_backward_data_x3(const void* dHs3, const void* hs3, void* dpre3, void* dh03, const void* wpack3T,
                                 const int32_t* tile_nodes, const int32_t* tile_off, const void* ell_col4, int64_t entries,
                                 int64_t B, int64_t T, int64_t N, int64_t F, int64_t K, double uniform_w, const float* rank1, void* stream);
int gcrnn_fused_backward_weight_f32(const void* dpre3, const void* Xuser, const void* Huser, const void* h0user, float* dW,
                                    float* dbsum, const int32_t* tile_nodes, const int32_t* tile_off, const void* ell_col4,
                                    int64_t entries, int64_t B, int64_t T, int64_t N, int64_t F, int64_t G, int64_t K,
                                    double uniform_w, const float* rank1, void* stream);
int gcrnn_fused_backward_data_x3_gated(const void* dHs3, const void* hs3, void* dpre3, void* dh03, const void* wpack3T,
                                       const int32_t* tile_nodes, const int32_t* tile_off, const void* ell_col4, int64_t entries,
                                       int64_t B, int64_t T, int64_t N, int64_t F, int64_t K, double uniform_w, const float* gf,
                                       const void* h03, float* dgf_parts, const float* rank1, void* stream);
int gcrnn_fused_filter_x3(const void* z3, void* out3, const void* wpack3, const int32_t* tile_nodes, const int32_t* tile_off,
                          const void* ell_col4, int64_t entries, int64_t B, int64_t N, int64_t F, int64_t K, double uniform_w,
                          const float* rank1, void* stream);
int gcrnn_fused_backward_weight_f32_gated(const void* dpre3, const void* Xuser, const void* Huser, const void* h0user, float* dW,
                                          float* dbsum, const int32_t* tile_nodes, const int32_t* tile_off, const void* ell_col4,
                                          int64_t entries, int64_t B, int64_t T, int64_t N, int64_t F, int64_t G, int64_t K,
                                          double uniform_w, const float* gi, const float* gf, int h_is_h0, const float* rank1, void* stream);
int gcrnn_fused_gate_cells_x3(const void* xs3, const void* h03, void* scratch3, const void* wpack3, const float* bias,
                              const int32_t* tile_nodes, const int32_t* tile_off, const void* ell_col4, int64_t entries, int64_t B,
                              int64_t T, int64_t N, int64_t F, int64_t G, int64_t K, double uniform_w, void* Cuser, int state_zero, const float* rank1, void* stream);
int gcrnn_pack_seq_major_x3_ex(const void* src, void* dst, int64_t B, int64_t T, int64_t C, int64_t N, int64_t NPad,
                               const float* item_scale, const float* rowmul, int one_minus_square, int64_t src_seq_stride, void* stream);
int gcrnn_x3_item_dots(const void* a3, const void* b3, const float* vec, float* out_ab, float* out_av, int64_t B, int64_t T, int64_t NPad,
                       int64_t C, void* stream);
int gcrnn_x3_node_gate_step(const void* ya3, const void* yb3, const float* ni, const float* nf, const float* bias, void* h3, void* Huser,
                            int64_t huser_seq_stride, int64_t B, int64_t N, int64_t NPad, int64_t F, void* stream);


int gcrnn_ell_assign_rows(const int32_t* rowptr, const int32_t* col, int64_t N, const int32_t* order, int pad,
                          int64_t ntiles, int32_t* node_addr);
int gcrnn_ell_assign_rows_z(const int32_t* rowptr, const int32_t* col, int64_t N, const int32_t* order, int pad,
                            int64_t ntiles, int64_t zero_from, int32_t* node_addr);
int gcrnn_ell_fill_z(const int32_t* rowptr, const int32_t* col, const double* val, int64_t N, const int32_t* order,
                     int tile, int pad, int64_t ntiles, const int32_t* node_addr, int64_t zero_from, int32_t* tile_off,
                     int32_t* ell_col, float* ell_val);
int gcrnn_ell_conflict_cycles(const int32_t* ell_col, int64_t entries, const int32_t* node_addr, int64_t* cycles);
int gcrnn_ell_pack_lds(const int32_t* ell_col, const float* ell_val, int64_t entries, const int32_t* node_addr, float* val4,
                       uint16_t* col4);
int gcrnn_fused_supported(int64_t N, int64_t F, int64_t G, int64_t K);
int64_t gcrnn_fused_padded_nodes(void);
int64_t gcrnn_fused_step_waves(void);
int64_t gcrnn_fused_wgrad_waves(void);
int gcrnn_pack_seq_major(int dtype, const void* src, void* dst, int64_t B, int64_t T, int64_t C, int64_t N,
                         int64_t NPad, const int32_t* perm, void* stream);
int gcrnn_pack_seq_major_padded(const void* src, void* dst, int64_t B, int64_t T, int64_t Cs, int64_t C, int64_t N, int64_t NPad,
                                void* stream);
int gcrnn_unpack_seq_major(int dtype, const void* src, void* dst, int64_t B, int64_t T, int64_t C, int64_t N,
                           int64_t NPad, const int32_t* perm, void* stream);
int gcrnn_pack_seq_major_steps(const void* src, void* dst, int64_t B, int64_t T, int64_t C, int64_t N, int64_t NPad,
                               int64_t t0, int64_t t1, int64_t max_blocks ,
                               void* stream);
int gcrnn_fused_pack_weights(int wdtype, const void* wA, const void* wB, void* wpack, int64_t F, int64_t G,
                             int64_t Kin, int64_t Kst, void* stream);
int gcrnn_fused_inline_pack_supported(int64_t N, int64_t F, int64_t G, int64_t K, int64_t entries, double uniform_w);
int64_t gcrnn_fused_seq_steps_per_launch(int64_t B, int64_t T, int64_t N, int64_t F, int64_t G, int64_t K, int64_t entries,
                                         double uniform_w, int img16, int inline_pack, int backward);
int gcrnn_fused_forward_bf16(const void* xs, const void* h0, void* hs, const void* wpack, const float* bias,
                             const float* gi, const float* gf, const int32_t* tile_nodes, const int32_t* tile_off,
                             const int32_t* ell_col, const float* ell_val, const void* ell_val4, const void* ell_col4,
                             int64_t entries, int64_t B, int64_t T, int64_t N, int64_t F, int64_t G, int64_t K,
                             void* Huser, int huser_last_only, void* const* step_events, double uniform_w,
                             const void* Xuser_inline ,
                             const float* head_w ,
                             float* head_part ,
                             void* stream);

int gcrnn_fused_pack_weights_wide(int wdtype, const void* wA, const void* wB, void* wpack, int64_t Fout, int64_t F, int64_t G, int64_t Kin,
                                  int64_t Kst, double uniform_w, void* stream);
int gcrnn_fused_forward_wide_supported(int64_t B, int64_t T, int64_t N, int64_t F, int64_t G, int64_t K, int64_t entries, double uniform_w,
                                       int img16, int inline_pack);
int gcrnn_fused_forward_wide_bf16(const void* xs, const void* h0, void* hs, const void* wpack, const float* bias, const float* gi,
                                  const float* gf, const int32_t* tile_nodes, const int32_t* tile_off, const void* ell_col4, int64_t entries,
                                  int64_t B, int64_t T, int64_t N, int64_t F, int64_t G, int64_t K, void* Huser, int huser_last_only,
                                  const void* Xuser_inline,
                                  const float* rank1_a, const float* rank1_b ,
                                  void* stream);
int64_t gcrnn_fused_forward_wide_scratch_bytes(int64_t B, int64_t F, int rank1);
int gcrnn_fused_forward_wide_scratch_bf16(const void* xs, const void* h0, void* scratch, int64_t scratch_bytes, const void* wpack,
                                          const float* bias, const float* gi, const float* gf, const int32_t* tile_nodes,
                                          const int32_t* tile_off, const void* ell_col4, int64_t entries, int64_t B, int64_t T, int64_t N,
                                          int64_t F, int64_t G, int64_t K, void* Huser, int huser_last_only, const void* Xuser_inline,
                                          const float* rank1_a, const float* rank1_b, void* stream);
int gcrnn_fused_forward_wide_head_supported(int64_t B, int64_t T, int64_t N, int64_t F, int64_t G, int64_t K, int64_t entries, double uniform_w,
                                            int img16, int inline_pack);
int gcrnn_fused_forward_wide_head_bf16(const void* xs, const void* h0, void* scratch, int64_t scratch_bytes, const void* wpack,
                                       const float* bias, const float* gi, const float* gf, const int32_t* tile_nodes,
                                       const int32_t* tile_off, const void* ell_col4, int64_t entries, int64_t B, int64_t T, int64_t N,
                                       int64_t F, int64_t G, int64_t K, const float* head_w, const float* head_b, float* Y,
                                       const void* Xuser_inline, const float* rank1_a, const float* rank1_b, void* stream);
#define GCRNN_WIDE_SELF_START 2
int gcrnn_fused_pack_weights_wide_bias(int wdtype, const void* wA, const void* wB, const void* bias, void* wpack, float* bias_out, int64_t Fout,
                                       int64_t F, int64_t G, int64_t Kin, int64_t Kst, double uniform_w, void* stream);
int64_t gcrnn_fused_forward_wide_user_bytes(int64_t B, int64_t T, int64_t G);
int gcrnn_fused_forward_wide_user_supported(int64_t B, int64_t T, int64_t N, int64_t F, int64_t G, int64_t K, int64_t entries, double uniform_w,
                                            int img16);
int gcrnn_fused_forward_wide_user_bf16(void* xs_work, int64_t xs_bytes, const void* h0_user, void* scratch, int64_t scratch_bytes,
                                       const void* wpack, const float* bias, const int32_t* tile_nodes, const int32_t* tile_off,
                                       const void* ell_col4, int64_t entries, int64_t B, int64_t T, int64_t N, int64_t F, int64_t G, int64_t K,
                                       void* Huser, int huser_last_only, const void* Xuser, const float* rank1_a, const float* rank1_b,
                                       void* stream);
int gcrnn_fused_forward_wide_head_user_supported(int64_t B, int64_t T, int64_t N, int64_t F, int64_t G, int64_t K, int64_t entries,
                                                 double uniform_w, int img16);
int gcrnn_fused_forward_wide_head_user_bf16(void* xs_work, int64_t xs_bytes, const void* h0_user, void* scratch, int64_t scratch_bytes,
                                            const void* wpack, const float* bias, const int32_t* tile_nodes, const int32_t* tile_off,
                                            const void* ell_col4, int64_t entries, int64_t B, int64_t T, int64_t N, int64_t F, int64_t G,
                                            int64_t K, const float* head_w, const float* head_b, float* Y, const void* Xuser,
                                            const float* rank1_a, const float* rank1_b, void* stream);
int gcrnn_fused_gate_pair_wide_supported(int64_t B, int64_t T, int64_t N, int64_t F, int64_t G, int64_t K, int64_t entries, double uniform_w,
                                         int img16, int with_pack);
int gcrnn_fused_backward_data_wide_supported(int64_t B, int64_t T, int64_t N, int64_t F, int64_t K, int64_t entries, double uniform_w, int img16,
                                             int inline_pack);
int gcrnn_fused_backward_data_wide_bf16(const void* dHs, const void* hs, void* dpre, void* dh0, const void* wpackT, const int32_t* tile_nodes,
                                        const int32_t* tile_off, const void* ell_col4, int64_t entries, int64_t B, int64_t T, int64_t N,
                                        int64_t F, int64_t K, const float* gf, const void* h0s, float* dgf_parts, const void* dHuser_inline,
                                        const float* rank1_a, const float* rank1_b, void* stream);
int gcrnn_fused_backward_data_wide_head_supported(int64_t B, int64_t T, int64_t N, int64_t F, int64_t K, int64_t entries, double uniform_w,
                                                  int img16);
int gcrnn_fused_backward_data_wide_head_bf16(const void* dy, const float* w_head, const void* hs, void* dpre, void* dh0, const void* wpackT,
                                             const int32_t* tile_nodes, const int32_t* tile_off, const void* ell_col4, int64_t entries,
                                             int64_t B, int64_t T, int64_t N, int64_t F, int64_t K, const float* gf, const void* h0s,
                                             float* dgf_parts, void* stream);
int gcrnn_fused_filter_output_wide_supported(int64_t B, int64_t T, int64_t N, int64_t F, int64_t G, int64_t K, int64_t entries, double uniform_w,
                                             int img16, int with_pack );
int gcrnn_fused_filter_output_wide_bf16(const void* xs, const void* wpack, const float* bias, void* out, const int32_t* tile_nodes,
                                        const int32_t* tile_off, const void* ell_col4, int64_t entries, int64_t B, int64_t T, int64_t N,
                                        int64_t F, int64_t G, int64_t K,
                                        const void* x_user ,
                                        void* stream);
int gcrnn_fused_node_forward_wide_supported(int64_t B, int64_t T, int64_t N, int64_t F, int64_t K, int64_t entries, double uniform_w, int img16);
int gcrnn_fused_node_forward_wide_bf16(const void* h0s, void* hs, const void* yx, const float* ngates, const float* gi, const float* gf,
                                       const void* wpackB, const float* bias, const int32_t* tile_nodes, const int32_t* tile_off,
                                       const void* ell_col4, int64_t entries, int64_t B, int64_t T, int64_t N, int64_t F, int64_t K, void* Huser,
                                       int huser_last_only, void* stream);
int gcrnn_gate_readout_finish(const float* parts, int64_t nparts, const float* lb_in, const float* lb_f, float* gi, float* gf, int64_t items,
                              void* stream);
int gcrnn_fused_gate_pair_prepass_wide_bf16(const void* x_user, void* xs, const void* h0, const void* wpack, const float* bias2,
                                            const float* gw2, float* parts, void* cs_in, void* cs_f, const int32_t* tile_nodes,
                                            const int32_t* tile_off, const void* ell_col4, int64_t entries, int64_t B, int64_t T, int64_t N,
                                            int64_t F, int64_t G, int64_t K, const int32_t* h0_zero_flag, const float* rank1_a, const float* rank1_b,
                                            void* stream);
int gcrnn_fused_gate_pair_prepass_taps_wide_bf16(const void* x_user, void* xs, const void* h0, const void* wpack, const float* bias2,
                                                 const void* tapf, float* taps_out, int64_t ntaps, void* cs_in, void* cs_f,
                                                 const int32_t* tile_nodes, const int32_t* tile_off, const void* ell_col4, int64_t entries,
                                                 int64_t B, int64_t T, int64_t N, int64_t F, int64_t G, int64_t K, const int32_t* h0_zero_flag,
                                                 const float* rank1_a, const float* rank1_b, void* stream);

int gcrnn_fused_gate_prepass_bf16(const void* xs, const void* h0, const void* wpack, const float* bias,
                                  const float* gate_w, float* gate_out, void* cs, const int32_t* tile_nodes,
                                  const int32_t* tile_off, const int32_t* ell_col, const float* ell_val,
                                  const void* ell_val4, const void* ell_col4, int64_t entries, int64_t B, int64_t T,
                                  int64_t N, int64_t F, int64_t G, int64_t K, const int32_t* h0_zero_flag, double uniform_w,
                                  int img16 , void* stream);

int gcrnn_fused_gate_prepass_pack_bf16(const void* x_user, void* xs, const void* h0, const void* wpack, const float* bias,
                                       const float* gate_w, float* gate_out, void* cs, const int32_t* tile_nodes,
                                       const int32_t* tile_off, const int32_t* ell_col, const float* ell_val,
                                       const void* ell_val4, const void* ell_col4, int64_t entries, int64_t B, int64_t T,
                                       int64_t N, int64_t F, int64_t G, int64_t K, const int32_t* h0_zero_flag, double uniform_w,
                                       int img16, void* stream);
int64_t gcrnn_fused_gate_prepass_lays_out(int64_t B, int64_t T, int64_t N, int64_t F, int64_t G, int64_t K, int64_t entries,
                                          double uniform_w, int img16);

int gcrnn_fused_gate_prepass_taps_bf16(const void* x_user, void* xs, const void* h0, const void* wpack, const float* bias,
                                       const void* tap_frags, float* taps_out, int64_t ntaps, void* cs, const int32_t* tile_nodes,
                                       const int32_t* tile_off, const int32_t* ell_col, const float* ell_val, const void* ell_val4,
                                       const void* ell_col4, int64_t entries, int64_t B, int64_t T, int64_t N, int64_t F, int64_t G,
                                       int64_t K, const int32_t* h0_zero_flag, double uniform_w, int img16, void* stream);
int gcrnn_fused_gate_prepass_taps_supported(int64_t B, int64_t T, int64_t N, int64_t F, int64_t G, int64_t K, int64_t entries,
                                            double uniform_w, int img16, int with_pack, int64_t ntaps);

int gcrnn_fused_gate_grad_bf16(const void* zs, const void* xs, const void* dpre, const void* wpack, const float* bias, float* out,
                               const int32_t* tile_nodes, const int32_t* tile_off, const int32_t* ell_col, const float* ell_val,
                               const void* ell_val4, const void* ell_col4, int64_t entries, int64_t B, int64_t T, int64_t N,
                               int64_t F, int64_t G, int64_t K, double uniform_w ,
                               int img16 , void* stream);

int64_t gcrnn_fused_gate_readout_slabs(int64_t items);
int gcrnn_all_zero_flag_bf16(const void* src, int64_t elements, int32_t* flag, void* stream);
int gcrnn_fused_gate_readout_backward_bf16(void* cs, const float* dlogit, const float* gate_w, float* dw_part, int64_t items,
                                           int64_t N, int64_t F, void* stream);

int gcrnn_fused_backward_data_bf16(const void* dHs, const void* hs, void* dpre, void* dh0, const void* wpackT,
                                   const int32_t* tile_nodes, const int32_t* tile_off, const int32_t* ell_col,
                                   const float* ell_val, const void* ell_val4, const void* ell_col4, int64_t entries,
                                   int64_t B, int64_t T, int64_t N, int64_t F, int64_t K, const float* gf, const void* h0s,
                                   float* dgf_parts, double uniform_w,
                                   const void* dHuser_inline ,
                                   int img16 ,
                                   void* stream);

int64_t gcrnn_fused_wgrad_slots(int64_t items, int64_t F);
int64_t gcrnn_fused_wgrad_bf16_slots(int64_t items, int64_t F, int64_t K, int64_t entries, int img16);
int gcrnn_fused_backward_weight_bf16(const void* dpre, const void* Xuser, const void* Huser, const void* h0user, float* dW,
                                     float* dbsum ,
                                     const int32_t* tile_nodes, const int32_t* tile_off, const void* ell_val4,
                                     const void* ell_col4, int64_t entries, int64_t B, int64_t T, int64_t N, int64_t F,
                                     int64_t G, int64_t K, const float* gi, const float* gf, int h_is_h0,
                                     const int32_t* h0_zero_flag ,
                                     double uniform_w ,
                                     const float* rank1_a, const float* rank1_b ,
                                     void* stream);

int gcrnn_small_supported(int dtype, int64_t N, int64_t nnz, int64_t G, int64_t F, int64_t Kin, int64_t Kst);
int gcrnn_small_forward(int dtype, const void* X, const void* h0, const void* wA, const void* wB, const void* bias,
                        const void* gi, const void* gf, const int32_t* rowptr, const int32_t* col, const void* val,
                        void* H, int64_t B, int64_t T, int64_t N, int64_t G, int64_t F, int64_t Kin, int64_t Kst,
                        int64_t nnz, void* stream);

int gcrnn_small_backward_supported(int dtype, int64_t N, int64_t nnz, int64_t G, int64_t F, int64_t Kin, int64_t Kst);
int gcrnn_small_backward(int dtype, const void* X, const void* h0, const void* H, const void* dH, const void* wA,
                         const void* wB, const void* bias, const void* gi, const void* gf, const int32_t* rowptr,
                         const int32_t* col, const void* val, const int32_t* arowptr, const int32_t* acol, const void* aval,
                         void* pA, void* pB, void* pb, void* dgi, void* dgf, void* dh0, int64_t B, int64_t T, int64_t N,
                         int64_t G, int64_t F, int64_t Kin, int64_t Kst, int64_t nnz, void* stream);
int gcrnn_small_backward_dx(int dtype, const void* X, const void* h0, const void* H, const void* dH, const void* wA,
                            const void* wB, const void* bias, const void* gi, const void* gf, const int32_t* rowptr,
                            const int32_t* col, const void* val, const int32_t* arowptr, const int32_t* acol, const void* aval,
                            void* pA, void* pB, void* pb, void* dgi, void* dgf, void* dh0, void* dX, int64_t B, int64_t T,
                            int64_t N, int64_t G, int64_t F, int64_t Kin, int64_t Kst, int64_t nnz, void* stream);

int gcrnn_small_dense_supported(int dtype, int64_t N, int64_t G, int64_t F, int64_t Kin, int64_t Kst, int backward,
                                int gated);
int gcrnn_small_dense_forward(int dtype, const void* X, const void* h0, const void* wA, const void* wB, const void* bias,
                              const void* gi, const void* gf, const void* Sdense, void* H, int64_t B, int64_t T, int64_t N,
                              int64_t G, int64_t F, int64_t Kin, int64_t Kst, int64_t gate_stride_b, int64_t gate_stride_t,
                              int64_t gate_stride_n, void* stream);
int gcrnn_small_dense_backward(int dtype, const void* X, const void* h0, const void* H, const void* dH, const void* wA,
                               const void* wB, const void* bias, const void* gi, const void* gf, const void* Sdense,
                               void* pA, void* pB, void* pb, void* dgi, void* dgf, void* dh0, int64_t B, int64_t T,
                               int64_t N, int64_t G, int64_t F, int64_t Kin, int64_t Kst, int64_t gate_stride_b,
                               int64_t gate_stride_t, int64_t gate_stride_n, void* stream);
int gcrnn_small_dense_backward_dx_supported(int dtype, int64_t N, int64_t G, int64_t F, int64_t Kin, int64_t Kst, int gated);
int gcrnn_small_dense_backward_dx(int dtype, const void* X, const void* h0, const void* H, const void* dH, const void* wA,
                                  const void* wB, const void* bias, const void* gi, const void* gf, const void* Sdense,
                                  void* pA, void* pB, void* pb, void* dgi, void* dgf, void* dh0, void* dX, int64_t B, int64_t T,
                                  int64_t N, int64_t G, int64_t F, int64_t Kin, int64_t Kst, int64_t gate_stride_b,
                                  int64_t gate_stride_t, int64_t gate_stride_n, void* stream);

#define GCRNN_SMALL_HEAD_MAX_CLASSES 1024
enum { GCRNN_SMALL_STATES_ALL = 0, GCRNN_SMALL_STATES_LAST = 1, GCRNN_SMALL_STATES_NONE = 2 };
int gcrnn_small_dense_head_supported(int dtype, int64_t N, int64_t G, int64_t F, int64_t Kin, int64_t Kst, int64_t C,
                                     int backward, int gated, int dx);
int gcrnn_small_dense_forward_head(int dtype, const void* X, const void* h0, const void* wA, const void* wB, const void* bias,
                                   const void* gi, const void* gf, const void* Sdense, const void* head_w, const void* head_b,
                                   void* H, void* logits, int64_t B, int64_t T, int64_t N, int64_t G, int64_t F, int64_t Kin,
                                   int64_t Kst, int64_t gate_stride_b, int64_t gate_stride_t, int64_t gate_stride_n, int64_t C,
                                   int store_states, void* stream);
int gcrnn_small_dense_backward_head(int dtype, const void* X, const void* h0, const void* H, const void* dlogits,
                                    const void* head_w, const void* wA, const void* wB, const void* bias, const void* gi,
                                    const void* gf, const void* Sdense, void* pA, void* pB, void* pb, void* dgi, void* dgf,
                                    void* dh0, void* dX, int64_t B, int64_t T, int64_t N, int64_t G, int64_t F, int64_t Kin,
                                    int64_t Kst, int64_t gate_stride_b, int64_t gate_stride_t, int64_t gate_stride_n, int64_t C,
                                    void* stream);

#define GCRNN_SMALL_NODE_HEAD_MAX_OUT 8
int gcrnn_small_dense_node_head_supported(int dtype, int64_t N, int64_t G, int64_t F, int64_t Kin, int64_t Kst, int64_t O,
                                          int backward, int gated, int dx);
int gcrnn_small_dense_forward_node_head(int dtype, const void* X, const void* h0, const void* wA, const void* wB, const void* bias,
                                        const void* gi, const void* gf, const void* Sdense, const void* node_w, const void* node_b,
                                        void* H, void* Y, int64_t B, int64_t T, int64_t N, int64_t G, int64_t F, int64_t Kin,
                                        int64_t Kst, int64_t gate_stride_b, int64_t gate_stride_t, int64_t gate_stride_n, int64_t O,
                                        int store_states, void* stream);
int gcrnn_small_dense_backward_node_head(int dtype, const void* X, const void* h0, const void* H, const void* dY,
                                         const void* node_w, const void* wA, const void* wB, const void* bias, const void* gi,
                                         const void* gf, const void* Sdense, void* pA, void* pB, void* pb, void* dgi, void* dgf,
                                         void* dh0, void* dX, int64_t B, int64_t T, int64_t N, int64_t G, int64_t F, int64_t Kin,
                                         int64_t Kst, int64_t gate_stride_b, int64_t gate_stride_t, int64_t gate_stride_n, int64_t O,
                                         void* stream);

int gcrnn_small_dense_gnn_head_supported(int dtype, int64_t N, int64_t G, int64_t F, int64_t Kin, int64_t Kst, int64_t K_o,
                                         int backward, int gated, int dx);
int gcrnn_small_dense_forward_gnn_head(int dtype, const void* X, const void* h0, const void* wA, const void* wB, const void* bias,
                                       const void* gi, const void* gf, const void* Sdense, const void* head_w, const void* head_b,
                                       void* H, void* Y, int64_t B, int64_t T, int64_t N, int64_t G, int64_t F, int64_t Kin,
                                       int64_t Kst, int64_t gate_stride_b, int64_t gate_stride_t, int64_t gate_stride_n, int64_t K_o,
                                       int act, int store_states, void* stream);
int gcrnn_small_gnn_head_adjoint(int dtype, const void* dY, const void* Y, const void* Sdense, void* dU, int64_t items, int64_t N,
                                 int64_t K_o, int act, void* stream);

int gcrnn_small_gates_supported(int dtype, int64_t N, int64_t G, int64_t F, int64_t Kin, int64_t Kst, int backward);
int gcrnn_small_gates_forward(int dtype, const void* X, const void* h0, const void* wA2, const void* wB2, const void* bias2,
                              const void* lw2, const void* lb2, const void* Sdense, void* gate, int64_t B, int64_t T,
                              int64_t N, int64_t G, int64_t F, int64_t Kin, int64_t Kst, void* stream);
int gcrnn_small_gates_backward(int dtype, const void* X, const void* h0, const void* wA2, const void* wB2, const void* bias2,
                               const void* lw2, const void* Sdense, const void* dsum, void* pA, void* pB, void* pb, void* plw,
                               void* plb, void* pdh0, int64_t B, int64_t T, int64_t N, int64_t G, int64_t F, int64_t Kin,
                               int64_t Kst, void* stream);
int gcrnn_small_gates_backward_dx(int dtype, const void* X, const void* h0, const void* wA2, const void* wB2, const void* bias2,
                                  const void* lw2, const void* Sdense, const void* dsum, void* pA, void* pB, void* pb, void* plw,
                                  void* plb, void* pdh0, void* pdX, int64_t B, int64_t T, int64_t N, int64_t G, int64_t F,
                                  int64_t Kin, int64_t Kst, void* stream);

int gcrnn_small_node_gates_supported(int dtype, int64_t N, int64_t G, int64_t F, int64_t Kin, int64_t Kst, int backward);
int gcrnn_small_node_gates_forward(int dtype, const void* X, const void* h0, const void* wA2, const void* wB2, const void* bias2,
                                   const void* wf2, const void* bf2, const void* Sdense, void* gate, int64_t B, int64_t T,
                                   int64_t N, int64_t G, int64_t F, int64_t Kin, int64_t Kst, void* stream);
int gcrnn_small_node_gates_backward(int dtype, const void* X, const void* h0, const void* wA2, const void* wB2, const void* bias2,
                                    const void* wf2, const void* Sdense, const void* dl, void* pA, void* pB, void* pb, void* pwf,
                                    void* pbf, void* pdh0, int64_t B, int64_t T, int64_t N, int64_t G, int64_t F, int64_t Kin,
                                    int64_t Kst, void* stream);
int gcrnn_small_node_gates_backward_dx(int dtype, const void* X, const void* h0, const void* wA2, const void* wB2,
                                       const void* bias2, const void* wf2, const void* Sdense, const void* dl, void* pA, void* pB,
                                       void* pb, void* pwf, void* pbf, void* pdh0, void* pdX, int64_t B, int64_t T, int64_t N,
                                       int64_t G, int64_t F, int64_t Kin, int64_t Kst, void* stream);

int gcrnn_small_edge_supported(int dtype, int64_t N, int64_t nnz, int64_t nnz_support, int64_t G, int64_t F, int64_t Kin,
                               int64_t Kst);
int gcrnn_small_edge_forward(int dtype, const void* X, const void* h0, const void* wA, const void* wB, const void* bias,
                             const void* att_in_w, const void* att_in_a, const void* att_f_w, const void* att_f_a, const void* gi,
                             const void* gf, const int32_t* rowptr, const int32_t* col, const void* val, const int32_t* s_rowptr,
                             const int32_t* r_edge, const int32_t* t_rowptr, const int32_t* t_edge, const void* t_val, void* Ya,
                             void* H, int64_t B, int64_t T, int64_t N, int64_t G, int64_t F, int64_t Kin, int64_t Kst, int64_t nnz,
                             int64_t nnz_support, int last_only, void* stream);

int gcrnn_small_edge_backward_supported(int dtype, int64_t N, int64_t nnz, int64_t nnz_support, int64_t G, int64_t F, int64_t Kin,
                                        int64_t Kst);
int gcrnn_small_edge_backward(int dtype, const void* X, const void* h0, const void* H, const void* dH, const void* wA,
                              const void* wB, const void* bias, const void* att_in_w, const void* att_in_a, const void* att_f_w,
                              const void* att_f_a, const void* gi, const void* gf, const int32_t* rowptr, const int32_t* col,
                              const void* val, const int32_t* a_rowptr, const int32_t* a_col, const void* a_val,
                              const int32_t* s_rowptr, const int32_t* r_edge, const int32_t* t_rowptr, const int32_t* t_edge,
                              const void* t_val, const int32_t* t_pos, void* dPre, void* pwfA, void* pbfA, void* pwfB, void* pbfB,
                              void* dgi, void* dgf, void* dh0, int64_t B, int64_t T, int64_t N, int64_t G, int64_t F, int64_t Kin,
                              int64_t Kst, int64_t nnz, int64_t nnz_support, void* stream);
int gcrnn_small_edge_backward_dx(int dtype, const void* X, const void* h0, const void* H, const void* dH, const void* wA,
                                 const void* wB, const void* bias, const void* att_in_w, const void* att_in_a, const void* att_f_w,
                                 const void* att_f_a, const void* gi, const void* gf, const int32_t* rowptr, const int32_t* col,
                                 const void* val, const int32_t* a_rowptr, const int32_t* a_col, const void* a_val,
                                 const int32_t* s_rowptr, const int32_t* r_edge, const int32_t* t_rowptr, const int32_t* t_edge,
                                 const void* t_val, const int32_t* t_pos, void* dPre, void* pwfA, void* pbfA, void* pwfB, void* pbfB,
                                 void* dgi, void* dgf, void* dh0, void* dX, int64_t B, int64_t T, int64_t N, int64_t G, int64_t F,
                                 int64_t Kin, int64_t Kst, int64_t nnz, int64_t nnz_support, void* stream);

enum { GCRNN_SMALL_EDGE_HEAD_LAST = 1, GCRNN_SMALL_EDGE_HEAD_NODE = 2 };
int gcrnn_small_edge_head_supported(int dtype, int64_t N, int64_t nnz, int64_t nnz_support, int64_t G, int64_t F, int64_t Kin,
                                    int64_t Kst, int head_kind, int64_t NC, int backward);
int gcrnn_small_edge_forward_head(int dtype, const void* X, const void* h0, const void* wA, const void* wB, const void* bias,
                                  const void* att_in_w, const void* att_in_a, const void* att_f_w, const void* att_f_a, const void* gi,
                                  const void* gf, const int32_t* rowptr, const int32_t* col, const void* val, const int32_t* s_rowptr,
                                  const int32_t* r_edge, const int32_t* t_rowptr, const int32_t* t_edge, const void* t_val, void* Ya,
                                  void* H, const void* head_w, const void* head_b, void* Y, int64_t B, int64_t T, int64_t N, int64_t G,
                                  int64_t F, int64_t Kin, int64_t Kst, int64_t nnz, int64_t nnz_support, int64_t NC, int head_kind,
                                  int store_states, void* stream);
int gcrnn_small_edge_backward_head(int dtype, const void* X, const void* h0, const void* H, const void* up, const void* head_w,
                                   const void* wA, const void* wB, const void* bias, const void* att_in_w, const void* att_in_a,
                                   const void* att_f_w, const void* att_f_a, const void* gi, const void* gf, const int32_t* rowptr,
                                   const int32_t* col, const void* val, const int32_t* a_rowptr, const int32_t* a_col, const void* a_val,
                                   const int32_t* s_rowptr, const int32_t* r_edge, const int32_t* t_rowptr, const int32_t* t_edge,
                                   const void* t_val, const int32_t* t_pos, void* dPre, void* pwfA, void* pbfA, void* pwfB, void* pbfB,
                                   void* dgi, void* dgf, void* dh0, void* dX, int64_t B, int64_t T, int64_t N, int64_t G, int64_t F,
                                   int64_t Kin, int64_t Kst, int64_t nnz, int64_t nnz_support, int64_t NC, int head_kind, void* stream);

int64_t gcrnn_node_linear_blocks(int64_t R, int64_t N);
int gcrnn_node_linear_forward(int dtype, const void* h, const void* w, const void* b, void* y, int64_t R, int64_t N, int64_t F,
                              int64_t O, void* stream);
int gcrnn_node_linear_backward(int dtype, const void* h, const void* w, const void* dy, void* dh, void* pw, void* pb, int64_t R,
                               int64_t N, int64_t F, int64_t O, void* stream);

int gcrnn_node_linear_bf16_supported(int64_t N, int64_t F, int64_t O);
int64_t gcrnn_node_linear_bf16_blocks(int64_t R, int64_t N);
int gcrnn_node_linear_bf16_forward(int wdtype, const void* h, const void* w, const void* b, void* y, int64_t R, int64_t N,
                                   int64_t F, int64_t O, void* stream);
int gcrnn_node_linear_bf16_backward(int wdtype, const void* h, const void* w, const void* dy, void* dh, float* pw, float* pb,
                                    int64_t R, int64_t N, int64_t F, int64_t O, void* stream);

int gcrnn_graph_filter_layer_supported(int dtype, int64_t N, int64_t nnz, int64_t E, int64_t F_in, int64_t F_out, int64_t K,
                                       int uniform);
int64_t gcrnn_graph_filter_layer_wgrad_slots(int dtype, int64_t items, int64_t N, int64_t nnz, int64_t F_in, int64_t F_out,
                                             int64_t K, int uniform);
int gcrnn_graph_filter_layer_forward(int dtype, const void* x, const void* w, const void* b, void* y, const int32_t* rowptr,
                                     const int32_t* col, const void* val, double uniform_w, int64_t items, int64_t N, int64_t nnz,
                                     int64_t E, int64_t F_in, int64_t F_out, int64_t K, int act, void* stream);
int gcrnn_graph_filter_layer_backward(int dtype, const void* x, const void* w, const void* y, const void* dy, void* dx,
                                      void* dw_parts, void* db_parts, int64_t slots, const int32_t* rowptr, const int32_t* col,
                                      const void* val, double uniform_w, int64_t items, int64_t N, int64_t nnz, int64_t E,
                                      int64_t F_in, int64_t F_out, int64_t K, int act, void* stream);

int gcrnn_rnn_supported(int dtype, int64_t B, int64_t T, int64_t D, int64_t F_h);
int64_t gcrnn_rnn_wgrad_slots(int dtype, int64_t B, int64_t T, int64_t D, int64_t F_h);
int gcrnn_rnn_forward(int dtype, const void* x, const void* h0, const void* w_ih, const void* w_hh, const void* b_ih,
                      const void* b_hh, void* H, int64_t B, int64_t T, int64_t D, int64_t F_h, int act, void* stream);
int gcrnn_rnn_backward(int dtype, const void* x, const void* h0, const void* w_ih, const void* w_hh, const void* H, const void* dH,
                       void* dZ, void* dh0, void* dx, void* dw_parts, int64_t slots, int64_t B, int64_t T, int64_t D, int64_t F_h,
                       int act, void* stream);

int64_t gcrnn_l1_loss_blocks(int64_t n);
int gcrnn_l1_loss(int dtype, const void* x, const void* y, void* grad, void* partial, int64_t n, double inv_n, void* stream);
int gcrnn_scale_unless_one(int dtype, void* data, const void* r, int64_t n, void* stream);
int64_t gcrnn_batch_time_mse_slabs(int64_t R, int64_t C);
int gcrnn_batch_time_mse(int dtype, const void* x, const void* y, void* part, void* out, int64_t R, int64_t C, void* stream);
#define GCRNN_CROSS_ENTROPY_MAX_CLASSES 1024
int64_t gcrnn_cross_entropy_blocks(int64_t B, int64_t C);
int gcrnn_cross_entropy(int dtype, const void* logits, const int64_t* labels, void* grad, void* partial, int64_t* hit_partial,
                        void* loss_out, int64_t* hits_out, int64_t B, int64_t C, double inv_B, void* stream);

int gcrnn_adam_flat(int dtype, void* p, const void* g, void* m, void* v, int64_t n, double lr, double beta1, double beta2,
                    double eps, double grad_scale, int64_t* step_dev, void* stream);
int gcrnn_adam_flat_dlr(int dtype, void* p, const void* g, void* m, void* v, int64_t n, const double* lr_dev, double beta1,
                        double beta2, double eps, double grad_scale, int64_t* step_dev, void* stream);
int gcrnn_sgd_flat(int dtype, void* p, const void* g, int64_t n, const double* lr_dev, double grad_scale, void* stream);
int gcrnn_rmsprop_flat(int dtype, void* p, const void* g, void* v, int64_t n, const double* lr_dev, double alpha, double eps,
                       double grad_scale, void* stream);

int gcrnn_attention_forward(int dtype, const int32_t* rowptr, const int32_t* col, const void* val, const int32_t* t_rowptr,
                            const int32_t* t_row, const int32_t* t_pos, const void* Wx, const void* s1, const void* s2,
                            void* alpha, void* y, int64_t T, int64_t N, int64_t B, int64_t F, int64_t nnz,
                            double negative_slope, void* stream);
int gcrnn_attention_backward(int dtype, const int32_t* rowptr, const int32_t* col, const void* val,
                             const int32_t* edge_row , const int32_t* t_rowptr, const int32_t* t_pos, const void* Wx, const void* s1, const void* s2,
                             const void* alpha, const void* dy, void* dWx, void* ds1, void* ds2, void* dz_scratch, int64_t T,
                             int64_t N, int64_t B, int64_t F, int64_t nnz, double negative_slope, void* stream);

#ifdef __cplusplus
}
#endif
#endif
```

Before: 167,100.

## Keep part of the state chunk resident in LDS via a three-slot weight ring

Replaces the full per-chunk weight buffer in LDS with a 3-slot rotating ring of per-tap weight blocks. The freed LDS holds up to RT of each wave's state tiles from the first chunk, so the second chunk reads them from LDS instead of the global scratch buffer. A new launcher picks RT=3 or 2 from what fits in LDS and routes the inline-pack, un-gated self-start forward to it. This cuts scratch round trips to global memory, at the cost of extra weight DMA issues per hop and ring-slot bookkeeping.

New measurement: 170,200 (median of 6 runs). 1.8% higher.

```diff
diff --git a/gated_gcrnns_amd/_lib.py b/gated_gcrnns_amd/_lib.py
--- a/gated_gcrnns_amd/_lib.py
+++ b/gated_gcrnns_amd/_lib.py
@@ -89,6 +89,7 @@
         'gcrnn_fused_forward_wide_head_bf16': (C.c_int, [_c_p] * 3 + [_c_i64] + [_c_p] * 7 + [_c_i64] * 7 + [_c_p] * 7),
         'gcrnn_fused_pack_weights_wide_bias': (C.c_int, [C.c_int] + [_c_p] * 5 + [_c_i64] * 5 + [C.c_double, _c_p]),
         'gcrnn_fused_forward_wide_user_bytes': (_c_i64, [_c_i64] * 3),
+        'gcrnn_fused_forward_wide_resident_tiles': (C.c_int, [_c_i64] * 4 + [C.c_int]),
         'gcrnn_fused_forward_wide_user_supported': (C.c_int, [_c_i64] * 7 + [C.c_double, C.c_int]),
         'gcrnn_fused_forward_wide_user_bf16': (C.c_int, [_c_p, _c_i64, _c_p, _c_p, _c_i64] + [_c_p] * 5 + [_c_i64] * 7 + [_c_p, C.c_int, _c_p, _c_p, _c_p, _c_p]),
         'gcrnn_fused_forward_wide_head_user_supported': (C.c_int, [_c_i64] * 7 + [C.c_double, C.c_int]),
diff --git a/gated_gcrnns_amd/csrc/gcrnn_fused_seq32.h b/gated_gcrnns_amd/csrc/gcrnn_fused_seq32.h
--- a/gated_gcrnns_amd/csrc/gcrnn_fused_seq32.h
+++ b/gated_gcrnns_amd/csrc/gcrnn_fused_seq32.h
@@ -131,7 +131,7 @@
     }                                                                                              \
   } while (0)
 
-template <int K, int HS, int XS>
+template <int K, int HS, int XS, int RT = 0>
 struct Seq32Map {
   static constexpr int KS = HS + XS;
   static constexpr int PL = GCRNN_HOP_WIDE_PLANE;
@@ -139,11 +139,18 @@
   static constexpr int BIAS_OFF = PL + 32 * 1024;
   static constexpr int FLAG_OFF = BIAS_OFF + 256;
   static constexpr int WOFF = 2 * PL;
-  static constexpr int WB = K * KS * 2048;
-  static constexpr int COL_OFF = WOFF + WB;
+  static constexpr int RING = RT > 0 ? 3 : K;
+  static constexpr int TAPB = KS * 2048;
+  static constexpr int WCH = K * TAPB;
+  static constexpr int WB = RING * TAPB;
+  static constexpr int RES_OFF = WOFF + WB;
+  static constexpr int RES_B = RT * (HS - 1) * SWAVES * 1024;
+  static constexpr int COL_OFF = RES_OFF + RES_B;
   static constexpr int NPCK = 128;
   static constexpr int PFS = 256;
   static_assert(16 * RS2 <= BIAS_OFF && FLAG_OFF + 768 <= WOFF, "LDS map");
+  static_assert(RT >= 0 && RT <= STILES && (RT == 0 || HS > 1), "resident tiles: a share of a wave's tiles, of a state with a re-read chunk");
+  static_assert(WOFF + RING * TAPB == RES_OFF && RES_OFF + RES_B == COL_OFF && RES_OFF % 1024 == 0, "LDS map: ring, resident block, column words");
   static size_t lds_bytes(int64_t entries, bool inline_pack, bool r1 = false) {
     const size_t need = (size_t)COL_OFF + (size_t)entries * 32 + GCRNN_HOP_COLUMN_PAD + NP * 4 + (r1 ? 2 * NP * 4 : 0) + (inline_pack ? (size_t)(32 * (XS > 0 ? XS : HS)) * NPCK * 2 : 0)
                         + PFS;
@@ -156,7 +163,7 @@
   }
 };
 
-template <int K, int HS, int XS, int VAR, int MODE = 0, bool GATED = false, bool R1 = false, bool SPLIT = false>
+template <int K, int HS, int XS, int VAR, int MODE = 0, bool GATED = false, bool R1 = false, bool SPLIT = false, int RT = 0>
 __global__ __launch_bounds__(STHREADS) void fused_seq32_kernel(const Seq32Args a) {
   static_assert(!R1 || !SPLIT, "rank-1 graphs: every mode of the persistent form (the BPTT chain takes the adjoint plan: the factors swap)");
   static_assert(!SPLIT || ((MODE == 0 || MODE == 2) && !R1 && HS > 1), "split sequences: the (un-gated or time-gated) forward and the BPTT chain, with more than one chunk");
@@ -172,11 +179,13 @@
   constexpr int SCR_CH = NP * 64;
   static_assert(MODE == 0 || ((MODE >= 1 && MODE <= 4) && !GATED), "modes");
   static_assert(MODE < 3 || (!R1 && !SPLIT), "modes 3, 4: uniform-weight graphs, persistent form");
-  using M = Seq32Map<K, HS, XS>;
+  using M = Seq32Map<K, HS, XS, RT>;
+  constexpr bool RINGV = RT > 0;
+  static_assert(!RINGV || (VAR == 7 && MODE == 0 && !GATED && !SPLIT && HS > 1), "resident tiles: the un-gated self-start forward, more than one chunk");
   constexpr int KS = HS + XS;
   constexpr int F = 32 * HS, G = 32 * XS;
   constexpr int NCH = (MODE == 1) ? 2 * HS : HS;
-  constexpr int PL = M::PL, WOFF = M::WOFF, WB = M::WB, COL_OFF = M::COL_OFF, RS2 = M::RS2;
+  constexpr int PL = M::PL, WOFF = M::WOFF, WCH = M::WCH, TAPB = M::TAPB, COL_OFF = M::COL_OFF, RS2 = M::RS2;
   constexpr int NPCK = M::NPCK, NRND = NP / NPCK, NH = NCH * (K - 1), RPH = (NRND + NH - 1) / NH;
   constexpr int PKROWS = SONLY ? F : G;
   static_assert(STILES == 8 && GCRNN_HOP_ASM && K >= 2 && (SONLY ? XS == 0 : XS > 0), "generated hop stream: 8 tiles per wave; the chain's operand is the state alone");
@@ -332,6 +341,15 @@
     }
   };
 
+  [[maybe_unused]] auto ring_start = [&]() {
+    const char* w0 = reinterpret_cast<const char*>(a.wpack);
+    const int ln = lane_now();
+    for (int p = wave; p < 2 * (TAPB / 1024); p += SWAVES) {
+      const int item = p / (TAPB / 1024), piece = p - item * (TAPB / 1024);
+      __builtin_amdgcn_global_load_lds((const __attribute__((address_space(1))) void*)(w0 + (K - 1 - item) * TAPB + piece * 1024 + ln * 16),
+                                       (__attribute__((address_space(3))) void*)(smem + WOFF + p * 1024), 16, 0, 0);
+    }
+  };
   {
     const int cbytes = entries * 32;
     const char* csrc = reinterpret_cast<const char*>(a.ell_col4);
@@ -339,8 +357,10 @@
       if (p * 1024 + lane * 16 < cbytes)
         __builtin_amdgcn_global_load_lds((const __attribute__((address_space(1))) void*)(csrc + p * 1024 + lane * 16),
                                          (__attribute__((address_space(3))) void*)(smem + COL_OFF + p * 1024), 16, 0, 0);
-    const char* wsrc = reinterpret_cast<const char*>(a.wpack) + (size_t)chunk0 * WB;
-    for (int p = wave; p < WB / 1024; p += SWAVES)
+    const char* wsrc = reinterpret_cast<const char*>(a.wpack) + (size_t)chunk0 * WCH;
+    if constexpr (RINGV) ring_start();
+    else
+    for (int p = wave; p < WCH / 1024; p += SWAVES)
       __builtin_amdgcn_global_load_lds((const __attribute__((address_space(1))) void*)(wsrc + p * 1024 + lane * 16),
                                        (__attribute__((address_space(3))) void*)(smem + WOFF + p * 1024), 16, 0, 0);
     asm volatile("s_waitcnt vmcnt(0)" ::: "memory");
@@ -392,6 +412,13 @@
   };
   bool have_operand = self_start;
   for (int b = wg_seq; b < B; b += gseq) {
+  if constexpr (RINGV) {
+    if (b != wg_seq) {
+      ring_start();
+      asm volatile("s_waitcnt vmcnt(0)" ::: "memory");
+      lds_barrier();
+    }
+  }
   if (!have_operand) load_first_operand(b);
   have_operand = false;
 #pragma unroll 1
@@ -434,12 +461,16 @@
     const __amdgpu_buffer_rsrc_t rsrc_xn = __builtin_amdgcn_make_buffer_rsrc(const_cast<uint16_t*>(XS > 0 ? a.x0 + (int64_t)(step + 1) * a.xstride : nullptr), 0, (more && XS > 0) ? B * (NP * G * 2) : 0, 0x00020000);
 
     f32x4 acc[STILES][2];
-    auto taps = [&](int tap, [[maybe_unused]] bool on_sums = false) {
+    auto tap_off = [&](int ch, int tap) -> uint32_t {
+      if constexpr (RINGV) return ((uint32_t)((step * NCH + ch) * K + (K - 1 - tap)) % 3u) * (uint32_t)TAPB;
+      else return (uint32_t)(tap * TAPB);
+    };
+    auto taps = [&](int ch, int tap, [[maybe_unused]] bool on_sums = false) {
 #ifdef GCRNN_SEQ32_EXPERIMENT_NO_HOP_TAPS
       if (tap != K - 1) return;
 #endif
       const int ln = lane_now();
-      const uint32_t wofs = (uint32_t)WOFF + (uint32_t)ln * 16u;
+      const uint32_t wofs = (uint32_t)WOFF + (uint32_t)ln * 16u + tap_off(ch, tap);
       if constexpr (GATED) {
         const bool xpart = gin > 1e-30f;
         const bool hpart = !on_sums || gfo > 1e-30f;
@@ -453,7 +484,7 @@
           if (hpart) {
 #pragma unroll
             for (int s = 0; s < HS; ++s) {
-              const bf16x8 afr = __builtin_bit_cast(bf16x8, *reinterpret_cast<const uint4*>(smem + wofs + (uint32_t)(((tap * 2 + h) * KS + s) * 1024)));
+              const bf16x8 afr = __builtin_bit_cast(bf16x8, *reinterpret_cast<const uint4*>(smem + wofs + (uint32_t)((h * KS + s) * 1024)));
 #pragma unroll
               for (int i = 0; i < STILES; ++i) acc[i][h] = __builtin_amdgcn_mfma_f32_16x16x32_bf16(afr, bfr[i][s], acc[i][h], 0, 0, 0);
             }
@@ -465,7 +496,7 @@
           if (xpart) {
 #pragma unroll
             for (int s = HS; s < KS; ++s) {
-              const bf16x8 afr = __builtin_bit_cast(bf16x8, *reinterpret_cast<const uint4*>(smem + wofs + (uint32_t)(((tap * 2 + h) * KS + s) * 1024)));
+              const bf16x8 afr = __builtin_bit_cast(bf16x8, *reinterpret_cast<const uint4*>(smem + wofs + (uint32_t)((h * KS + s) * 1024)));
 #pragma unroll
               for (int i = 0; i < STILES; ++i) acc[i][h] = __builtin_amdgcn_mfma_f32_16x16x32_bf16(afr, bfr[i][s], acc[i][h], 0, 0, 0);
             }
@@ -481,17 +512,17 @@
 #pragma unroll
           for (int s = 0; s < KS; ++s) {
             if (s < HS && skip_h) continue;
-            const bf16x8 afr = __builtin_bit_cast(bf16x8, *reinterpret_cast<const uint4*>(smem + wofs + (uint32_t)(((tap * 2 + h) * KS + s) * 1024)));
+            const bf16x8 afr = __builtin_bit_cast(bf16x8, *reinterpret_cast<const uint4*>(smem + wofs + (uint32_t)((h * KS + s) * 1024)));
 #pragma unroll
             for (int i = 0; i < STILES; ++i) acc[i][h] = __builtin_amdgcn_mfma_f32_16x16x32_bf16(afr, bfr[i][s], acc[i][h], 0, 0, 0);
           }
       } else {
       uint4 af[2];
-      af[0] = *reinterpret_cast<const uint4*>(smem + wofs + (uint32_t)((tap * 2 * KS) * 1024));
+      af[0] = *reinterpret_cast<const uint4*>(smem + wofs);
 #pragma unroll
       for (int hs = 0; hs < 2 * KS; ++hs) {
         const int h = hs / KS, s = hs - h * KS;
-        if (hs + 1 < 2 * KS) af[(hs + 1) & 1] = *reinterpret_cast<const uint4*>(smem + wofs + (uint32_t)((tap * 2 * KS + hs + 1) * 1024));
+        if (hs + 1 < 2 * KS) af[(hs + 1) & 1] = *reinterpret_cast<const uint4*>(smem + wofs + (uint32_t)((hs + 1) * 1024));
         const bf16x8 afr = __builtin_bit_cast(bf16x8, af[hs & 1]);
 #pragma unroll
         for (int i = 0; i < STILES; ++i) acc[i][h] = __builtin_amdgcn_mfma_f32_16x16x32_bf16(afr, bfr[i][s], acc[i][h], 0, 0, 0);
@@ -517,18 +548,18 @@
         }
       }
     };
-    auto seed = [&]() {
+    auto seed = [&](int ch) {
 #pragma unroll
       for (int i = 0; i < STILES; ++i) { acc[i][0] = f32x4{0.f, 0.f, 0.f, 0.f}; acc[i][1] = f32x4{0.f, 0.f, 0.f, 0.f}; }
-      taps(K - 1);
+      taps(ch, K - 1);
       put(std::false_type{});
     };
-    auto seed_taps_beside_rows = [&]() {
+    auto seed_taps_beside_rows = [&](int ch) {
 #pragma unroll
       for (int i = 0; i < STILES; ++i) { acc[i][0] = f32x4{0.f, 0.f, 0.f, 0.f}; acc[i][1] = f32x4{0.f, 0.f, 0.f, 0.f}; }
-      taps(K - 1);
+      taps(ch, K - 1);
     };
-    seed();
+    seed(chunk0);
 
 #pragma unroll 1
     for (int chunk = chunk0; chunk < (SPLIT ? chunk0 + 1 : NCH); ++chunk) {
@@ -630,16 +661,21 @@
       };
 
       auto r0_of = [&](int j) { return (chunk * (K - 1) + (j - 1)) * RPH; };
-      auto weights_issue = [&](int wc, int tap) {
-        const char* wsrc = reinterpret_cast<const char*>(a.wpack) + (size_t)wc * WB + (size_t)tap * (2 * KS * 1024);
+      auto weights_issue = [&](int wc, int tap, uint32_t dst = 0xffffffffu) {
+        if (dst == 0xffffffffu) dst = (uint32_t)(tap * TAPB);
+        const char* wsrc = reinterpret_cast<const char*>(a.wpack) + (size_t)wc * WCH + (size_t)tap * (2 * KS * 1024);
         const int lane = lane_now();
 #pragma unroll
         for (int i = 0; i < (2 * KS + SWAVES - 1) / SWAVES; ++i) {
           const int piece = i * SWAVES + wave;
           if (piece < 2 * KS)
             __builtin_amdgcn_global_load_lds((const __attribute__((address_space(1))) void*)(wsrc + piece * 1024 + lane * 16),
-                                             (__attribute__((address_space(3))) void*)(smem + WOFF + tap * (2 * KS * 1024) + piece * 1024), 16, 0, 0);
-        }
+                                             (__attribute__((address_space(3))) void*)(smem + WOFF + dst + piece * 1024), 16, 0, 0);
+        }
+      };
+      [[maybe_unused]] auto ring_issue = [&](int pos) {
+        const int nx = pos >= K ? 1 : 0;
+        weights_issue(nx ? (chunk + 1) % NCH : chunk, K - 1 - (pos - nx * K), ((uint32_t)((step * NCH + chunk) * K + pos) % 3u) * (uint32_t)TAPB);
       };
       typedef __attribute__((__vector_size__(4 * sizeof(unsigned int)))) unsigned int u32x4e_t;
       [[maybe_unused]] u32x4e_t eph[MODE == 2 ? STILES : 1], epg[(SONLY && !UPR1) ? STILES : 1];
@@ -690,6 +726,10 @@
       auto hop = [&](auto jc) __attribute__((always_inline)) {
         constexpr int j = decltype(jc)::value;
         auto dma_issue = [&]() {
+          if constexpr (RINGV) {
+            if (j == 1) ring_issue(2);
+            ring_issue(j + 2);
+          } else
           if (NCH > 1 && !SPLIT) {
             weights_issue((chunk + 1) % NCH, K - j);
             if (j == 1 && K > 2) weights_issue(chunk, 0);
@@ -706,9 +746,9 @@
           r1_scale(acc, 0);
           GCRNN_STAMP32(1 + chunk * 24 + 4 * (j - 1) + 1);
           if (j == 2 && chunk == 0) GCRNN_STAMP32_WAVE(56);
-          taps(K - 1 - j, true);
+          taps(chunk, K - 1 - j, true);
         } else {
-          taps(K - 1 - j);
+          taps(chunk, K - 1 - j);
           r1_scale(acc, 1);
           if (j == 2 && chunk == 0) GCRNN_STAMP32_WAVE(56);
           dma_issue();
@@ -736,7 +776,7 @@
         if constexpr (R1 && j == K - 1) {
           if (!stream_first) r1_scale(acc, 2);
         }
-        if (K == 2 && NCH > 1 && !SPLIT) weights_issue((chunk + 1) % NCH, 0);
+        if (K == 2 && NCH > 1 && !SPLIT && !RINGV) weights_issue((chunk + 1) % NCH, 0);
         if (r0 < NRND) pack_drain(r0);
 #pragma unroll
         for (int e = 1; e < RPH; ++e) {
@@ -778,7 +818,9 @@
 #ifdef GCRNN_SEQ32_EXPERIMENT_SKIP
             if ((GCRNN_SEQ32_EXPERIMENT_SKIP == 1) == (s < HS)) continue;
 #endif
-            if (SCRV && s < HS)
+            if (RINGV && s < HS && i < RT)
+              bfr[i][s] = *reinterpret_cast<const bf16x8*>(smem + M::RES_OFF + ((s * SWAVES + wave) * RT + i) * 1024 + lane_now() * 16);
+            else if (SCRV && s < HS)
               bfr[i][s] = __builtin_bit_cast(bf16x8, __builtin_amdgcn_raw_buffer_load_b128(rsrc_sn, (lane_now() & 15) * 64 + 16 * qo, s * SCR_CH + (wave * STILES + i) * 1024, 16));
             else if (s < HS)
               bfr[i][s] = __builtin_bit_cast(bf16x8, __builtin_amdgcn_raw_buffer_load_b128(rsrc_hn, (w >> 16) * (F * 2) + 16 * qo + 64 * s, b * (NP * F * 2), GCRNN_SEQ32_NT_XLOAD));
@@ -986,7 +1028,10 @@
           }
         }
         if constexpr (SCRV) {
-          if (!last) __builtin_amdgcn_raw_buffer_store_b128(p, scratch_rsrc(), (lane & 15) * 64 + 16 * q, chunk * SCR_CH + (wave * STILES + i) * 1024, 0);
+          if (!last) {
+            if (RINGV && i < RT) *reinterpret_cast<u32x4_t*>(smem + M::RES_OFF + ((chunk * SWAVES + wave) * RT + i) * 1024 + lane * 16) = p;
+            else __builtin_amdgcn_raw_buffer_store_b128(p, scratch_rsrc(), (lane & 15) * 64 + 16 * q, chunk * SCR_CH + (wave * STILES + i) * 1024, 0);
+          }
         } else
         if (GCRNN_SEQ32_NT_STATE && last) __builtin_amdgcn_raw_buffer_store_b128(p, rsrc_o, node * (F * 2) + (chunk * 32 + q * 8) * 2, b * (NP * F * 2), GCRNN_SEQ32_NT_STATE);
         else __builtin_amdgcn_raw_buffer_store_b128(p, rsrc_o, node * (F * 2) + (chunk * 32 + q * 8) * 2, b * (NP * F * 2), 0);
@@ -1010,6 +1055,7 @@
         for (int i = 0; i < STILES; ++i) bfr[i][HS - 1] = __builtin_bit_cast(bf16x8, pkd[i]);
       }
       if (GCRNN_SEQ32_OPERAND_AT == 1) request_next_operand();
+      GCRNN_STAMP32(1 + chunk * 24 + 22);
       if constexpr (ITEMS) {
         if (last && b + (int)gridDim.x < B && !GCRNN_SEQ32_NO_ITEM_PREFETCH) {
           load_first_operand(b + (int)gridDim.x);
@@ -1033,7 +1079,7 @@
       constexpr bool OVL = USERV && MODE == 0 && !GATED && !SPLIT;
       const bool ovl = OVL && chunk + 1 < NCH;
       if (ovl && wave < SWAVES / 2) {
-        seed_taps_beside_rows();
+        seed_taps_beside_rows(chunk + 1);
         GCRNN_STAMP32(1 + chunk * 24 + 21);
       }
       if (aux1) {
@@ -1069,16 +1115,16 @@
           }
         }
       }
-      if (ovl && wave >= SWAVES / 2) seed_taps_beside_rows();
+      if (ovl && wave >= SWAVES / 2) seed_taps_beside_rows(chunk + 1);
       if (GCRNN_SEQ32_OPERAND_AT == 2) request_next_operand();
       GCRNN_STAMP32(1 + chunk * 24 + 19);
-      if (K == 2 && NCH > 1 && !SPLIT) asm volatile("s_waitcnt vmcnt(0)" ::: "memory");
+      if (K == 2 && NCH > 1 && !SPLIT && !RINGV) asm volatile("s_waitcnt vmcnt(0)" ::: "memory");
       else if (GCRNN_SEQ32_END_WAIT) asm volatile("s_waitcnt vmcnt(0)" ::: "memory");
       lds_barrier();
       GCRNN_STAMP32(1 + chunk * 24 + 20);
       if (!SPLIT && chunk + 1 < NCH) {
         if (ovl) put(std::false_type{});
-        else seed();
+        else seed(chunk + 1);
       }
     }
   }
diff --git a/gated_gcrnns_amd/csrc/gcrnn_fused_seq32r.hip b/gated_gcrnns_amd/csrc/gcrnn_fused_seq32r.hip
--- /dev/null
+++ b/gated_gcrnns_amd/csrc/gcrnn_fused_seq32r.hip
@@ -0,0 +1,67 @@
+#include <cstdlib>
+#include "gcrnn_fused_step.h"
+#define GCRNN_SEQ32_STAMP_READER_NAME gcrnn_debug_read_seq32r_stamps
+#include "gcrnn_fused_seq32.h"
+
+
+static int seq32_resident_max() {
+  const char* e = getenv("GCRNN_SEQ32_RESIDENT");
+  if (!e) return 3;
+  return e[0] == '0' ? 0 : (e[0] == '2' ? 2 : 3);
+}
+
+template <int K, int XS, bool R1, int RT>
+static int seq32r_launch_v(const Seq32Args& sa, size_t lds, hipStream_t st) {
+  auto sk = fused_seq32_kernel<K, 2, XS, 7, 0, false, R1, false, RT>;
+  if (hipFuncSetAttribute(reinterpret_cast<const void*>(sk), hipFuncAttributeMaxDynamicSharedMemorySize, (int)lds) != hipSuccess)
+    return GCRNN_ERR_LAUNCH;
+  GCRNN_PRE_LAUNCH();
+  sk<<<(unsigned)((sa.B < gcrnn_persistent_grid() || sa.self_start) ? sa.B : gcrnn_persistent_grid()), STHREADS, lds, st>>>(sa);
+  GCRNN_CHECK_LAUNCH();
+  return GCRNN_OK;
+}
+
+size_t gcrnn_seq32r_lds(int K, int HS, int XS, int64_t entries, bool r1, int* rt) {
+  *rt = 0;
+  const int mx = seq32_resident_max();
+  if (HS != 2 || mx == 0) return 0;
+  if (K == 4 && XS == 2 && r1) return 0;
+#define GCRNN_SEQ32R_CASE(KK, XX) \
+  if (K == KK && XS == XX) { \
+    size_t l = mx >= 3 ? Seq32Map<KK, 2, XX, 3>::lds_bytes(entries, true, r1) : 0; \
+    if (l) { *rt = 3; return l; } \
+    l = Seq32Map<KK, 2, XX, 2>::lds_bytes(entries, true, r1); \
+    if (l) *rt = 2; \
+    return l; \
+  }
+  GCRNN_SEQ32R_CASE(5, 2) GCRNN_SEQ32R_CASE(4, 2) GCRNN_SEQ32R_CASE(3, 2) GCRNN_SEQ32R_CASE(2, 2)
+  GCRNN_SEQ32R_CASE(5, 1) GCRNN_SEQ32R_CASE(4, 1) GCRNN_SEQ32R_CASE(3, 1) GCRNN_SEQ32R_CASE(2, 1)
+#undef GCRNN_SEQ32R_CASE
+  return 0;
+}
+
+extern "C" int gcrnn_fused_forward_wide_resident_tiles(int64_t F, int64_t G, int64_t K, int64_t entries, int rank1) {
+  if (F != 64 || G <= 0 || G % 32 || entries <= 0) return 0;
+  int rt = 0;
+  gcrnn_seq32r_lds((int)K, 2, (int)(G / 32), entries, rank1 != 0, &rt);
+  return rt;
+}
+
+template <int K, int XS, bool R1>
+static int seq32r_launch_rt(const Seq32Args& sa, int rt, size_t lds, hipStream_t st) {
+  return rt == 3 ? seq32r_launch_v<K, XS, R1, 3>(sa, lds, st) : seq32r_launch_v<K, XS, R1, 2>(sa, lds, st);
+}
+
+int gcrnn_seq32r_forward(const Seq32Args& sa, int K, int XS, int rt, size_t lds, hipStream_t st) {
+  if (!sa.a1 || !sa.scr || sa.gi0 || !sa.pk_src0) return GCRNN_ERR_NULL_POINTER;
+  if (rt != 2 && rt != 3) return GCRNN_ERR_UNSUPPORTED;
+#define GCRNN_SEQ32R_CASE(KK, XX) \
+  if (K == KK && XS == XX) { \
+    if constexpr (KK == 4 && XX == 2) return sa.r1a ? GCRNN_ERR_UNSUPPORTED : seq32r_launch_rt<KK, XX, false>(sa, rt, lds, st); \
+    else return sa.r1a ? seq32r_launch_rt<KK, XX, true>(sa, rt, lds, st) : seq32r_launch_rt<KK, XX, false>(sa, rt, lds, st); \
+  }
+  GCRNN_SEQ32R_CASE(5, 2) GCRNN_SEQ32R_CASE(4, 2) GCRNN_SEQ32R_CASE(3, 2) GCRNN_SEQ32R_CASE(2, 2)
+  GCRNN_SEQ32R_CASE(5, 1) GCRNN_SEQ32R_CASE(4, 1) GCRNN_SEQ32R_CASE(3, 1) GCRNN_SEQ32R_CASE(2, 1)
+#undef GCRNN_SEQ32R_CASE
+  return GCRNN_ERR_UNSUPPORTED;
+}
diff --git a/gated_gcrnns_amd/csrc/gcrnn_fused_seq32s.hip b/gated_gcrnns_amd/csrc/gcrnn_fused_seq32s.hip
--- a/gated_gcrnns_amd/csrc/gcrnn_fused_seq32s.hip
+++ b/gated_gcrnns_amd/csrc/gcrnn_fused_seq32s.hip
@@ -14,9 +14,17 @@
   return GCRNN_OK;
 }
 
+size_t gcrnn_seq32r_lds(int K, int HS, int XS, int64_t entries, bool r1, int* rt);
+int gcrnn_seq32r_forward(const Seq32Args& sa, int K, int XS, int rt, size_t lds, hipStream_t st);
+
 template <int K, int HS, int XS>
 static int seq32s_launch(const Seq32Args& sa, bool inline_pack, size_t lds, hipStream_t st) {
   if (!sa.a1 || (HS > 1 && !sa.scr)) return GCRNN_ERR_NULL_POINTER;
+  if (HS > 1 && inline_pack && !sa.gi0) {
+    int rt = 0;
+    const size_t ldsr = gcrnn_seq32r_lds(K, HS, XS, sa.entries, sa.r1a != nullptr, &rt);
+    if (ldsr) return gcrnn_seq32r_forward(sa, K, XS, rt, ldsr, st);
+  }
   if (sa.gi0) {
     if (inline_pack) return GCRNN_ERR_BAD_SHAPE;
     return sa.r1a ? seq32s_launch_v<K, HS, XS, 6, true, true>(sa, lds, st) : seq32s_launch_v<K, HS, XS, 6, true, false>(sa, lds, st);
diff --git a/include/gcrnn.h b/include/gcrnn.h
--- a/include/gcrnn.h
+++ b/include/gcrnn.h
@@ -214,6 +214,7 @@
                                        int64_t F, int64_t G, int64_t K, const float* head_w, const float* head_b, float* Y,
                                        const void* Xuser_inline, const float* rank1_a, const float* rank1_b, void* stream);
 #define GCRNN_WIDE_SELF_START 2
+int gcrnn_fused_forward_wide_resident_tiles(int64_t F, int64_t G, int64_t K, int64_t entries, int rank1);
 int gcrnn_fused_pack_weights_wide_bias(int wdtype, const void* wA, const void* wB, const void* bias, void* wpack, float* bias_out, int64_t Fout,
                                        int64_t F, int64_t G, int64_t Kin, int64_t Kst, double uniform_w, void* stream);
 int64_t gcrnn_fused_forward_wide_user_bytes(int64_t B, int64_t T, int64_t G);
```
